# dalek-cryptography/zkp

Measured on AMD Instinct MI355X. Metric: proofs/sec + batch-verifies/sec, CMZ13 10-attr credential, 1/2/4/8 MI355X, higher is better.
Workload: dtype u32x9 (29-bit limbs, u64 accumulate)

## Files before the change

### zkp_amd/csrc/comb_tables.h

```cpp
#pragma once
#include "quad.h"
#include "stmt_pairs.h"

namespace zkp {

template <int TEETH>
struct comb_cfg {
  static_assert(TEETH == 4 || TEETH == 8 || TEETH == 16 || TEETH == 32, "teeth");
  static constexpr int BITS = 256 / TEETH;
  static constexpr int WINDOWS = BITS / 4;
  static constexpr int ENTRIES = 8 * TEETH + 1;
};
constexpr int comb_entries(int teeth) { return 8 * teeth + 1; }
constexpr int LADDER_ENTRIES = 8;

__device__ __forceinline__ void q_store_cached(dev_ext* dst, const qcached& c, int q) {
  uint32_t* w = reinterpret_cast<uint32_t*>(dst) + 9 * q;
#pragma unroll
  for (int i = 0; i < 9; ++i) w[i] = c.c.v[i];
}

__global__ void __launch_bounds__(256)
k_comb_slots(uint32_t n_points, const uint32_t* __restrict__ uses, uint32_t comb_min, uint32_t group_min, uint32_t max_tables,
             uint32_t* __restrict__ counter, uint32_t* __restrict__ slot_of, uint32_t* __restrict__ slot_pt, uint32_t* __restrict__ group_start,
             dev_affine* __restrict__ pts) {
  const uint32_t pi = blockIdx.x * blockDim.x + threadIdx.x;
  const uint32_t u = pi < n_points ? uses[pi] : 0u;
  const bool want = pi < n_points && u >= comb_min;
  const uint64_t mask = __ballot(want);
  if (!mask) return;
  const uint32_t lane = threadIdx.x & 63u;
  const int leader = __ffsll((long long)mask) - 1;
  const uint32_t gu = (want && u >= group_min) ? u : 0u;
  uint32_t incl = gu;
#pragma unroll
  for (int d = 1; d < 64; d <<= 1) {
    const uint32_t up = (uint32_t)__shfl_up((int)incl, d);
    if ((int)lane >= d) incl += up;
  }
  const uint32_t total = (uint32_t)__shfl((int)incl, 63);
  uint32_t base = 0, gbase = 0;
  if ((int)lane == leader) {
    base = atomicAdd(counter, (uint32_t)__popcll(mask));
    if (total) gbase = atomicAdd(counter + 1, total);
  }
  base = (uint32_t)__shfl((int)base, leader);
  gbase = (uint32_t)__shfl((int)gbase, leader);
  if (want) {
    const uint32_t slot = base + (uint32_t)__popcll(mask & ((1ull << lane) - 1ull));
    slot_of[pi] = slot < max_tables ? slot : 0xffffffffu;
    if (slot < max_tables) slot_pt[slot] = pi;
    else pts[pi].valid = 0;
    if (gu) group_start[pi] = gbase + incl - gu;
  }
}

template <int TEETH>
__global__ void __launch_bounds__(256, 2)
k_comb_tables(const uint32_t* __restrict__ n_slots, uint32_t max_tables, const uint32_t* __restrict__ slot_pt,
              const dev_affine* __restrict__ pts, dev_ext* __restrict__ comb) {
  using cfg = comb_cfg<TEETH>;
  const uint32_t gt = blockIdx.x * blockDim.x + threadIdx.x;
  const uint32_t slot = gt >> 2;
  const int q = (int)(gt & 3u);
  const uint32_t ns = min(*n_slots, max_tables);
  if (slot >= ns) return;
  const uint32_t pi = slot_pt[slot];
  if (pi & STMT_ABSORBED) return;
  qpt base;
  {
    const uint32_t* w = reinterpret_cast<const uint32_t*>(pts + pi);
    fe one;
    fe_1(one);
#pragma unroll
    for (int i = 0; i < 9; ++i) base.c.v[i] = q == 0 ? w[i] : (q == 1 ? w[9 + i] : (q == 3 ? w[18 + i] : one.v[i]));
  }
  dev_ext* tbl = comb + (size_t)slot * cfg::ENTRIES;
#pragma unroll 1
  for (int j = 0; j < TEETH; ++j) {
    qpt m2, m3, m4, m;
    qcached c1, c;
    q_to_cached(c1, base, q);
    q_store_cached(tbl + 8 * j + 0, c1, q);
    q_double(m2, base, q);
    q_to_cached(c, m2, q); q_store_cached(tbl + 8 * j + 1, c, q);
    q_add_cached(m3, m2, c1, q);
    q_to_cached(c, m3, q); q_store_cached(tbl + 8 * j + 2, c, q);
    q_double(m4, m2, q);
    q_to_cached(c, m4, q); q_store_cached(tbl + 8 * j + 3, c, q);
    q_add_cached(m, m4, c1, q);
    q_to_cached(c, m, q); q_store_cached(tbl + 8 * j + 4, c, q);
    q_double(m, m3, q);
    q_to_cached(c, m, q); q_store_cached(tbl + 8 * j + 5, c, q);
    q_add_cached(m, m, c1, q);
    q_to_cached(c, m, q); q_store_cached(tbl + 8 * j + 6, c, q);
    q_double(base, m4, q);
    q_to_cached(c, base, q); q_store_cached(tbl + 8 * j + 7, c, q);
#pragma unroll 1
    for (int d = 0; d < cfg::BITS - 3; ++d) q_double(base, base, q);
  }
  qcached c;
  q_to_cached(c, base, q);
  q_store_cached(tbl + 8 * TEETH, c, q);
}

__device__ __forceinline__ void store_comb_entry(dev_ext* dst, const ge_cached& c) {
  uint32_t w[36];
  fe_get(w, c.YmX); fe_get(w + 9, c.YpX); fe_get(w + 18, c.Z2); fe_get(w + 27, c.T2d);
  store_vec<9>(dst, w);
}
__device__ __forceinline__ void store_entries_staged(uint32_t (*stage)[64], const uint32_t* live, uint32_t lane, dev_ext* __restrict__ tbl0 ,
                                                     uint32_t entries_per_table, uint32_t e, const ge_cached& c) {
  uint32_t w[36];
  fe_get(w, c.YmX); fe_get(w + 9, c.YpX); fe_get(w + 18, c.Z2); fe_get(w + 27, c.T2d);
#pragma unroll
  for (int i = 0; i < 36; ++i) stage[i][lane] = w[i];
  __builtin_amdgcn_wave_barrier();
#pragma unroll
  for (int i = 0; i < 9; ++i) {
    const uint32_t ch = (uint32_t)i * 64u + lane, t = ch / 9u, q = ch - 9u * t;
    if (live[t]) {
      const uint4 v = make_uint4(stage[4 * q][t], stage[4 * q + 1][t], stage[4 * q + 2][t], stage[4 * q + 3][t]);
      reinterpret_cast<uint4*>(tbl0 + (size_t)t * entries_per_table + e)[q] = v;
    }
  }
  __builtin_amdgcn_wave_barrier();
}
template <int TEETH>
__device__ __forceinline__ void comb_table_lane(uint32_t slot, const uint32_t* __restrict__ n_slots, uint32_t max_tables, const uint32_t* __restrict__ slot_pt,
                                                const dev_affine* __restrict__ pts, dev_ext* __restrict__ comb) {
  using cfg = comb_cfg<TEETH>;
  const uint32_t ns = min(*n_slots, max_tables);
  if (slot >= ns) return;
  if (slot_pt[slot] & STMT_ABSORBED) return;
  ge_p3 base;
  load_affine(base, pts + slot_pt[slot]);
  dev_ext* tbl = comb + (size_t)slot * cfg::ENTRIES;
#pragma unroll 1
  for (int j = 0; j < TEETH; ++j) {
    ge_p3 m2, m3, m4, m;
    ge_cached c1, c;
    ge_to_cached(c1, base);
    store_comb_entry(tbl + 8 * j + 0, c1);
    ge_double<true>(m2, base);
    ge_to_cached(c, m2); store_comb_entry(tbl + 8 * j + 1, c);
    ge_add_cached(m3, m2, c1);
    ge_to_cached(c, m3); store_comb_entry(tbl + 8 * j + 2, c);
    ge_double<true>(m4, m2);
    ge_to_cached(c, m4); store_comb_entry(tbl + 8 * j + 3, c);
    ge_add_cached(m, m4, c1);
    ge_to_cached(c, m); store_comb_entry(tbl + 8 * j + 4, c);
    ge_double<true>(m, m3);
    ge_to_cached(c, m); store_comb_entry(tbl + 8 * j + 5, c);
    ge_add_cached(m, m, c1);
    ge_to_cached(c, m); store_comb_entry(tbl + 8 * j + 6, c);
    ge_double<true>(base, m4);
    ge_to_cached(c, base); store_comb_entry(tbl + 8 * j + 7, c);
#pragma unroll 1
    for (int d = 0; d < cfg::BITS - 4; ++d) ge_double<false>(base, base);
    ge_double<true>(base, base);
  }
  ge_cached c;
  ge_to_cached(c, base);
  store_comb_entry(tbl + 8 * TEETH, c);
}
template <int TEETH>
__global__ void __launch_bounds__(256, 2)
k_comb_tables_lane(const uint32_t* __restrict__ n_slots, uint32_t max_tables, const uint32_t* __restrict__ slot_pt,
                   const dev_affine* __restrict__ pts, dev_ext* __restrict__ comb) {
  comb_table_lane<TEETH>(blockIdx.x * blockDim.x + threadIdx.x, n_slots, max_tables, slot_pt, pts, comb);
}


template <int TEETH>
__device__ __forceinline__ void comb_table_pc(uint32_t slot0, const uint32_t* __restrict__ n_slots, uint32_t max_tables, const uint32_t* __restrict__ slot_pt,
                                              const dev_affine* __restrict__ pts, dev_ext* __restrict__ comb, uint32_t* hand) {
  using cfg = comb_cfg<TEETH>;
  const uint32_t wave = threadIdx.x >> 6, lane = threadIdx.x & 63u;
  const uint32_t ns = min(*n_slots, max_tables);
  const uint32_t slot = slot0 + lane;
  const bool have = slot < ns && !(slot_pt[slot < ns ? slot : 0u] & STMT_ABSORBED);
  dev_ext* tbl = comb + (size_t)(have ? slot : 0u) * cfg::ENTRIES;
  if (wave == 0) {
    ge_p3 base;
    ge_identity(base);
    if (have) load_affine(base, pts + slot_pt[slot]);
#pragma unroll 1
    for (int j = 0; j < TEETH; ++j) {
      uint32_t* h = hand + (j & 1) * 36 * 64 + lane;
#pragma unroll
      for (int i = 0; i < 9; ++i) { h[64 * i] = base.X.v[i]; h[64 * (9 + i)] = base.Y.v[i]; h[64 * (18 + i)] = base.Z.v[i]; h[64 * (27 + i)] = base.T.v[i]; }
      __syncthreads();
#pragma unroll 1
      for (int d = 0; d < cfg::BITS - 1; ++d) ge_double<false>(base, base);
      ge_double<true>(base, base);
    }
    if (have) {
      ge_cached c;
      ge_to_cached(c, base);
      store_comb_entry(tbl + 8 * TEETH, c);
    }
  } else {
#pragma unroll 1
    for (int j = 0; j < TEETH; ++j) {
      __syncthreads();
      const uint32_t* h = hand + (j & 1) * 36 * 64 + lane;
      ge_p3 base, m2, m3, m4, m;
#pragma unroll
      for (int i = 0; i < 9; ++i) { base.X.v[i] = h[64 * i]; base.Y.v[i] = h[64 * (9 + i)]; base.Z.v[i] = h[64 * (18 + i)]; base.T.v[i] = h[64 * (27 + i)]; }
      FE_TRACK(fe_set_ub_tight(base.X); fe_set_ub_tight(base.Y); fe_set_ub_tight(base.Z); fe_set_ub_tight(base.T));
      ge_cached c1, c;
      ge_to_cached(c1, base);
      ge_double<true>(m2, base);
      ge_add_cached(m3, m2, c1);
      ge_double<true>(m4, m2);
      if (have) {
        store_comb_entry(tbl + 8 * j + 0, c1);
        ge_to_cached(c, m2); store_comb_entry(tbl + 8 * j + 1, c);
        ge_to_cached(c, m3); store_comb_entry(tbl + 8 * j + 2, c);
        ge_to_cached(c, m4); store_comb_entry(tbl + 8 * j + 3, c);
      }
      ge_add_cached(m, m4, c1);
      if (have) { ge_to_cached(c, m); store_comb_entry(tbl + 8 * j + 4, c); }
      ge_double<true>(m, m3);
      if (have) { ge_to_cached(c, m); store_comb_entry(tbl + 8 * j + 5, c); }
      ge_add_cached(m, m, c1);
      if (have) { ge_to_cached(c, m); store_comb_entry(tbl + 8 * j + 6, c); }
      ge_double<true>(m, m4);
      if (have) { ge_to_cached(c, m); store_comb_entry(tbl + 8 * j + 7, c); }
    }
  }
}

__device__ __forceinline__ void load_comb_entry(ge_cached& c, const dev_ext* src) {
  uint32_t w[36];
  load_vec<9>(w, src);
  fe_set(c.YmX, w); fe_set(c.YpX, w + 9); fe_set(c.Z2, w + 18); fe_set(c.T2d, w + 27);
}

template <bool CT>
__device__ __forceinline__ void comb_select(ge_cached& sel, const dev_ext* __restrict__ row, uint32_t mag) {
  ge_cached_identity(sel);
  if (CT) {
#pragma unroll 1
    for (uint32_t h = 0; h < 4; ++h) {
      ge_cached c0, c1;
      load_comb_entry(c0, row + 2 * h + 0);
      load_comb_entry(c1, row + 2 * h + 1);
      ge_cached_cmov(sel, c0, (uint32_t)(mag == 2 * h + 1));
      ge_cached_cmov(sel, c1, (uint32_t)(mag == 2 * h + 2));
    }
  } else if (mag) {
    load_comb_entry(sel, row + (mag - 1));
  }
}

template <bool CT, int TEETH>
__device__ __forceinline__ void term_comb(uint32_t t, const uint8_t* __restrict__ scalars, const dev_ext* __restrict__ tbl,
                                          dev_ext* __restrict__ partial, uint32_t* ecol, bool no_carry = false) {
  using cfg = comb_cfg<TEETH>;
  uint32_t s[8], e[8], top;
  load_vec<2>(s, scalars + 32 * (size_t)t);
  sc_add_pattern(e, top, s, 0x88888888u);
#pragma unroll
  for (int j = 0; j < 8; ++j) ecol[256 * j] = e[j];
  ge_p3 acc;
  ge_identity(acc);
  if (CT) {
    ge_cached n0, n1;
    load_comb_entry(n0, tbl + 0);
    load_comb_entry(n1, tbl + 1);
#pragma unroll 1
    for (int w = cfg::WINDOWS - 1; w >= 0; --w) {
      if (w != cfg::WINDOWS - 1) {
        ge_double4_flat(acc);
      }
#pragma unroll 1
      for (int j = 0; j < TEETH; ++j) {
        const int nidx = j * cfg::WINDOWS + w;
        const uint32_t nib = (ecol[256 * (nidx >> 3)] >> (4 * (nidx & 7))) & 15u;
        const uint32_t neg = (uint32_t)(nib < 8u);
        const uint32_t mag = neg ? 8u - nib : nib - 8u;
        const dev_ext* row = tbl + 8 * j;
        ge_cached sel;
        ge_cached_identity(sel);
        ge_cached_cmov(sel, n0, (uint32_t)(mag == 1));
        ge_cached_cmov(sel, n1, (uint32_t)(mag == 2));
#pragma unroll 1
        for (uint32_t h = 1; h < 4; ++h) {
          ge_cached c0, c1;
          load_comb_entry(c0, row + 2 * h + 0);
          load_comb_entry(c1, row + 2 * h + 1);
          ge_cached_cmov(sel, c0, (uint32_t)(mag == 2 * h + 1));
          ge_cached_cmov(sel, c1, (uint32_t)(mag == 2 * h + 2));
        }
        const dev_ext* next = (j + 1 < TEETH) ? row + 8 : tbl;
        load_comb_entry(n0, next + 0);
        load_comb_entry(n1, next + 1);
        ge_cached_cneg(sel, neg);
        if (w == cfg::WINDOWS - 1 && j == 0) ge_from_cached(acc, sel);
        else ge_add_cached(acc, acc, sel);
      }
    }
  } else {
#pragma unroll 1
    for (int w = cfg::WINDOWS - 1; w >= 0; --w) {
      if (w != cfg::WINDOWS - 1) {
        ge_double4(acc);
      }
#pragma unroll 1
      for (int j = 0; j < TEETH; ++j) {
        const int nidx = j * cfg::WINDOWS + w;
        const uint32_t nib = (ecol[256 * (nidx >> 3)] >> (4 * (nidx & 7))) & 15u;
        const uint32_t neg = (uint32_t)(nib < 8u);
        const uint32_t mag = neg ? 8u - nib : nib - 8u;
        ge_cached sel;
        comb_select<false>(sel, tbl + 8 * j, mag);
        ge_cached_cneg(sel, neg);
        if (w == cfg::WINDOWS - 1 && j == 0) ge_from_cached(acc, sel);
        else ge_add_cached(acc, acc, sel);
      }
    }
  }
  if (!no_carry) {
    ge_cached sel, c;
    ge_cached_identity(sel);
    load_comb_entry(c, tbl + 8 * TEETH);
    ge_cached_cmov(sel, c, top);
    ge_add_cached(acc, acc, sel);
  }
  store_ext(partial + t, acc);
}

__device__ __forceinline__ void ge_p3_dpp_from(ge_p3& r, const ge_p3& a, int ctrl_sel) {
  if (ctrl_sel == 0) { fe_dpp<ZKP_QP(1, 1, 3, 3)>(r.X, a.X); fe_dpp<ZKP_QP(1, 1, 3, 3)>(r.Y, a.Y); fe_dpp<ZKP_QP(1, 1, 3, 3)>(r.Z, a.Z); fe_dpp<ZKP_QP(1, 1, 3, 3)>(r.T, a.T); }
  else { fe_dpp<ZKP_QP(2, 2, 2, 2)>(r.X, a.X); fe_dpp<ZKP_QP(2, 2, 2, 2)>(r.Y, a.Y); fe_dpp<ZKP_QP(2, 2, 2, 2)>(r.Z, a.Z); fe_dpp<ZKP_QP(2, 2, 2, 2)>(r.T, a.T); }
}
template <int TEETH>
__device__ __forceinline__ void term_comb_split4(uint32_t t, uint32_t q, const uint8_t* __restrict__ scalars, const dev_ext* __restrict__ comb, uint32_t slot,
                                                 dev_ext* __restrict__ partial, uint32_t* ecol, bool no_carry = false) {
  using cfg = comb_cfg<TEETH>;
  static_assert(cfg::WINDOWS == 4, "one lane of the quad per window");
  typedef __attribute__((address_space(3))) volatile uint32_t lds_word;
  lds_word* stash = (lds_word*)(ecol + 256 * 8);
  stash[0] = slot;
  stash[256] = t;
  const dev_ext* __restrict__ tbl = comb + (size_t)slot * cfg::ENTRIES;
  uint32_t s[8], e[8], top;
  load_vec<2>(s, scalars + 32 * (size_t)t);
  sc_add_pattern(e, top, s, 0x88888888u);
#pragma unroll
  for (int j = 0; j < 8; ++j) ecol[256 * j] = e[j];
  stash[512] = top;
  ge_p3 acc;
  ge_identity(acc);
  {
    ge_cached n0, n1;
    load_comb_entry(n0, tbl + 0);
    load_comb_entry(n1, tbl + 1);
#pragma unroll 1
    for (int j = 0; j < TEETH; ++j) {
      const uint32_t nidx = (uint32_t)j * cfg::WINDOWS + q;
      const uint32_t nib = (ecol[256 * (nidx >> 3)] >> (4 * (nidx & 7))) & 15u;
      const uint32_t neg = (uint32_t)(nib < 8u);
      const uint32_t mag = neg ? 8u - nib : nib - 8u;
      const dev_ext* row = tbl + 8 * j;
      ge_cached sel;
      ge_cached_identity(sel);
      ge_cached_cmov(sel, n0, (uint32_t)(mag == 1));
      ge_cached_cmov(sel, n1, (uint32_t)(mag == 2));
#pragma unroll 1
      for (uint32_t h = 1; h < 4; ++h) {
        ge_cached c0, c1;
        load_comb_entry(c0, row + 2 * h + 0);
        load_comb_entry(c1, row + 2 * h + 1);
        ge_cached_cmov(sel, c0, (uint32_t)(mag == 2 * h + 1));
        ge_cached_cmov(sel, c1, (uint32_t)(mag == 2 * h + 2));
      }
      const dev_ext* next = (j + 1 < TEETH) ? row + 8 : tbl;
      load_comb_entry(n0, next + 0);
      load_comb_entry(n1, next + 1);
      ge_cached_cneg(sel, neg);
      if (j == 0) ge_from_cached(acc, sel);
      else ge_add_cached(acc, acc, sel);
    }
  }
  {
    ge_p3 d = acc;
    ge_double4(d);
    fe_pick(acc.X, d.X, (q & 1u) != 0); fe_pick(acc.Y, d.Y, (q & 1u) != 0); fe_pick(acc.Z, d.Z, (q & 1u) != 0); fe_pick(acc.T, d.T, (q & 1u) != 0);
    ge_p3 o;
    ge_p3_dpp_from(o, acc, 0);
    ge_cached c;
    ge_to_cached(c, o);
    ge_add_cached(d, acc, c);
    fe_pick(acc.X, d.X, (q & 1u) == 0); fe_pick(acc.Y, d.Y, (q & 1u) == 0); fe_pick(acc.Z, d.Z, (q & 1u) == 0); fe_pick(acc.T, d.T, (q & 1u) == 0);
    d = acc;
    ge_double4(d);
    ge_double4(d);
    fe_pick(acc.X, d.X, q == 2u); fe_pick(acc.Y, d.Y, q == 2u); fe_pick(acc.Z, d.Z, q == 2u); fe_pick(acc.T, d.T, q == 2u);
    ge_p3_dpp_from(o, acc, 1);
    ge_to_cached(c, o);
    ge_add_cached(d, acc, c);
    fe_pick(acc.X, d.X, q == 0u); fe_pick(acc.Y, d.Y, q == 0u); fe_pick(acc.Z, d.Z, q == 0u); fe_pick(acc.T, d.T, q == 0u);
  }
  if (!no_carry) {
    ge_cached sel, c;
    ge_cached_identity(sel);
    load_comb_entry(c, comb + (size_t)stash[0] * cfg::ENTRIES + 8 * TEETH);
    ge_cached_cmov(sel, c, stash[512]);
    ge_add_cached(acc, acc, sel);
  }
  if (q == 0u) store_ext(partial + stash[256], acc);
}

constexpr int GROUP_RUNS = 3, GROUP_ROW_CHUNKS = 8 * 9, GROUP_IDENT_ROW = GROUP_RUNS * GROUP_ROW_CHUNKS, GROUP_CHUNK_ROWS = GROUP_IDENT_ROW + 9;
constexpr int GROUP_LDS_UINT4 = GROUP_CHUNK_ROWS * 16 + (256 + 16 * GROUP_RUNS) / 4;
static_assert(GROUP_MIN_USES >= 8, "a column of 16 consecutive grouped terms must span at most GROUP_RUNS points");

__device__ __forceinline__ void comb_group_block(uint32_t i0, uint32_t n_g, const uint32_t* __restrict__ list_g, const uint8_t* __restrict__ scalars,
                                                 const uint32_t* __restrict__ pidx, const uint32_t* __restrict__ slot_of,
                                                 const dev_ext* __restrict__ comb, dev_ext* __restrict__ partial, uint4* lds) {
  using cfg = comb_cfg<16>;
  constexpr uint32_t NONE = 0xffffffffu;
  const uint32_t tid = threadIdx.x, col = tid & 15u, k = tid >> 4;
  const uint32_t i = i0 + col * 16 + k;
  const bool listed = i < n_g;
  uint32_t t = 0, slot = NONE;
  if (listed) { t = list_g[i]; slot = slot_of[pidx[t]]; }
  uint32_t* slots = reinterpret_cast<uint32_t*>(lds + GROUP_CHUNK_ROWS * 16);
  uint32_t* colslot = slots + 256;
  slots[k * 16 + col] = slot;
  if (k < (uint32_t)GROUP_RUNS) colslot[col * GROUP_RUNS + k] = NONE;
  if (k < 9) {
    uint32_t w[36];
#pragma unroll
    for (int q = 0; q < 36; ++q) w[q] = (q == 0 || q == 9) ? 1u : (q == 18 ? 2u : 0u);
    uint4 v = make_uint4(0, 0, 0, 0);
#pragma unroll
    for (int q = 0; q < 9; ++q) if (k == (uint32_t)q) v = make_uint4(w[4 * q], w[4 * q + 1], w[4 * q + 2], w[4 * q + 3]);
    lds[(GROUP_IDENT_ROW + k) * 16 + col] = v;
  }
  __syncthreads();
  uint32_t run = 0;
  bool first = true;
#pragma unroll
  for (uint32_t kk = 1; kk < 16; ++kk) {
    const bool change = slots[kk * 16 + col] != slots[(kk - 1) * 16 + col];
    if (kk <= k) { run += change ? 1u : 0u; if (kk == k) first = change; }
  }
  if (first && run < (uint32_t)GROUP_RUNS) colslot[col * GROUP_RUNS + run] = slot;
  __syncthreads();
  const bool live = listed && slot != NONE && run < (uint32_t)GROUP_RUNS;
  const uint4* src[GROUP_RUNS];
  bool have[GROUP_RUNS];
#pragma unroll
  for (int r = 0; r < GROUP_RUNS; ++r) {
    const uint32_t sr = colslot[col * GROUP_RUNS + r];
    have[r] = sr != NONE;
    src[r] = reinterpret_cast<const uint4*>(comb + (size_t)(have[r] ? sr : 0u) * cfg::ENTRIES) + k;
  }
  const bool tail = k < (uint32_t)(GROUP_ROW_CHUNKS - 64);
  typedef __attribute__((address_space(1))) const void* gptr_t;
  typedef __attribute__((address_space(3))) void* lptr_t;
  const uint32_t wave = (uint32_t)__builtin_amdgcn_readfirstlane((int)(tid >> 6));
  auto issue = [&](uint32_t row) {
#pragma unroll
    for (int r = 0; r < GROUP_RUNS; ++r) {
      const uint4* p = src[r] + (size_t)row * GROUP_ROW_CHUNKS;
      uint4* d = lds + (size_t)(r * GROUP_ROW_CHUNKS + 4 * wave) * 16;
#pragma unroll
      for (int m = 0; m < 4; ++m)
        if (have[r]) __builtin_amdgcn_global_load_lds((gptr_t)(p + 16 * m), (lptr_t)(d + 16 * 16 * m), 16, 0, 0);
      if (have[r] && tail) __builtin_amdgcn_global_load_lds((gptr_t)(p + 64), (lptr_t)(d + 16 * 64), 16, 0, 0);
    }
  };
  uint32_t dlo[cfg::WINDOWS], dhi[cfg::WINDOWS], top = 0;
  {
    uint32_t sc[8], e[8];
#pragma unroll
    for (int q = 0; q < 8; ++q) sc[q] = 0;
    if (live) load_vec<2>(sc, scalars + 32 * (size_t)t);
    sc_add_pattern(e, top, sc, 0x88888888u);
#pragma unroll
    for (int w = 0; w < cfg::WINDOWS; ++w) {
      uint32_t lo = 0, hi = 0;
#pragma unroll
      for (int m = 0; m < 4; ++m) {
        lo |= (((e[m] >> (4 * w)) & 0xfu) | ((e[m] >> (12 + 4 * w)) & 0xf0u)) << (8 * m);
        hi |= (((e[m + 4] >> (4 * w)) & 0xfu) | ((e[m + 4] >> (12 + 4 * w)) & 0xf0u)) << (8 * m);
      }
      dlo[w] = lo; dhi[w] = hi;
    }
  }
  ge_p3 acc, lo;
  ge_identity(acc);
  ge_identity(lo);
  issue(0);
  auto pick = [&](uint32_t& c0, uint32_t& c1, ge_cached& sel, uint32_t& neg) {
    const uint32_t nib = c0 & 15u;
    c0 = __builtin_amdgcn_alignbit(c1, c0, 4);
    c1 >>= 4;
    neg = (uint32_t)(nib < 8u);
    const uint32_t mag = neg ? 8u - nib : nib - 8u;
    const uint32_t row = mag ? run * GROUP_ROW_CHUNKS + (mag - 1u) * 9u : (uint32_t)GROUP_IDENT_ROW;
    const uint4* ent = lds + (size_t)row * 16 + col;
    uint32_t wd[36];
#pragma unroll
    for (int q = 0; q < 9; ++q) {
      const uint4 x = ent[q * 16];
      wd[4 * q + 0] = x.x; wd[4 * q + 1] = x.y; wd[4 * q + 2] = x.z; wd[4 * q + 3] = x.w;
    }
    fe_set(sel.YmX, wd); fe_set(sel.YpX, wd + 9); fe_set(sel.Z2, wd + 18); fe_set(sel.T2d, wd + 27);
  };
#pragma unroll 1
  for (int pass = 0; pass < 2; ++pass) {
    if (live && pass) { ge_double4(acc); ge_double4(lo); }
    uint32_t alo = pass ? dlo[2] : dlo[3], ahi = pass ? dhi[2] : dhi[3];
    uint32_t blo = pass ? dlo[0] : dlo[1], bhi = pass ? dhi[0] : dhi[1];
#pragma unroll 1
    for (int j = 0; j < 16; ++j) {
      asm volatile("s_waitcnt vmcnt(0)\n\ts_barrier" ::: "memory");
      ge_cached sel;
      uint32_t neg = 0;
      const bool first = pass == 0 && j == 0;
      if (live) {
        pick(alo, ahi, sel, neg);
        ge_cached_cneg(sel, neg);
        if (first) ge_from_cached(acc, sel);
        else ge_add_cached(acc, acc, sel);
        pick(blo, bhi, sel, neg);
      }
      lds_barrier();
      if (pass == 0 || j != 15) issue((uint32_t)((j + 1) & 15));
      if (live) {
        ge_cached_cneg(sel, neg);
        if (first) ge_from_cached(lo, sel);
        else ge_add_cached(lo, lo, sel);
      }
    }
  }
  if (live) {
    ge_double4(acc);
    ge_double4(acc);
    ge_cached c;
    ge_to_cached(c, lo);
    ge_add_cached(acc, acc, c);
  }
  if (live) {
    ge_cached sel, c;
    ge_cached_identity(sel);
    load_comb_entry(c, comb + (size_t)slot * cfg::ENTRIES + 8 * 16);
    ge_cached_cmov(sel, c, top);
    ge_add_cached(acc, acc, sel);
    store_ext(partial + t, acc);
  }
}

constexpr uint32_t XBAR_RUNS = 8;
constexpr uint32_t XBAR_HALF_TERMS = 31, XBAR_WAVE_TERMS = 2 * XBAR_HALF_TERMS, XBAR_BLOCK_TERMS = 4 * XBAR_WAVE_TERMS;
constexpr int XBAR_WAVE_UINT4 = 9 * 64;
constexpr int XBAR_LDS_UINT4 = 4 * XBAR_WAVE_UINT4;
static_assert(2 + (XBAR_WAVE_TERMS - 2) / GROUP_MIN_USES <= XBAR_RUNS, "a wavefront's consecutive grouped terms must span at most XBAR_RUNS points");
static_assert(2 + (XBAR_HALF_TERMS - 2) / GROUP_MIN_USES <= 4 && XBAR_HALF_TERMS <= 32,
              "the terms of one crossbar service group (a half of the wavefront) must span at most 4 points: sources 32 lanes apart never meet");

__device__ __forceinline__ void comb_group_xbar(uint32_t i0, uint32_t n_g, const uint32_t* __restrict__ list_g, const uint8_t* __restrict__ scalars,
                                                const uint32_t* __restrict__ pidx, const uint32_t* __restrict__ slot_of,
                                                const dev_ext* __restrict__ comb, dev_ext* __restrict__ partial, uint4* lds, bool no_carry = false) {
  using cfg = comb_cfg<16>;
  constexpr uint32_t NONE = 0xffffffffu;
  const uint32_t tid = threadIdx.x, lane = tid & 63u;
  const uint32_t wave = (uint32_t)__builtin_amdgcn_readfirstlane((int)(tid >> 6));
  if (i0 + wave * XBAR_WAVE_TERMS >= n_g) return;
  const uint32_t hl = lane & 31u;
  const uint32_t i = i0 + wave * XBAR_WAVE_TERMS + (lane >> 5) * XBAR_HALF_TERMS + hl;
  const bool listed = hl < XBAR_HALF_TERMS && i < n_g;
  uint32_t t = 0, slot = NONE;
  if (listed) { t = list_g[i]; slot = slot_of[pidx[t]]; }
  uint32_t cur = slot;
  const uint32_t left = (uint32_t)__shfl_up((int)cur, 1);
  if (hl == 31u) cur = left;
  const uint32_t before = (uint32_t)__shfl_up((int)cur, 1);
  const bool change = lane == 0u || (listed && slot != before);
  const uint64_t cm = __ballot(change);
  const uint32_t run = (uint32_t)__popcll(cm & ((2ull << lane) - 1ull)) - 1u;
  const bool live = listed && slot != NONE && run < XBAR_RUNS;
  int first = -1;
  {
    uint64_t mm = cm;
#pragma unroll
    for (uint32_t r = 0; r < XBAR_RUNS; ++r) {
      const int f = mm ? (int)__ffsll((long long)mm) - 1 : -1;
      if ((lane >> 3) == r) first = f;
      mm &= mm - 1ull;
    }
  }
  uint32_t hslot = (uint32_t)__shfl((int)slot, first < 0 ? 0 : first);
  if (first < 0) hslot = NONE;
  const bool have = hslot != NONE;
  const uint4* hsrc = reinterpret_cast<const uint4*>(comb + (size_t)(have ? hslot : 0u) * cfg::ENTRIES + (lane & 7u));
  typedef __attribute__((address_space(1))) const void* gptr_t;
  typedef __attribute__((address_space(3))) void* lptr_t;
  uint4* wlds = lds + (size_t)wave * XBAR_WAVE_UINT4;
  const uint4* mine = wlds + lane;
  auto issue = [&](uint32_t row) {
    const uint4* p = hsrc + (size_t)row * (8 * 9);
    if (have) {
#pragma unroll
      for (int q = 0; q < 9; ++q) __builtin_amdgcn_global_load_lds((gptr_t)(p + q), (lptr_t)(wlds + 64 * q), 16, 0, 0);
    }
  };
  uint32_t dlo[cfg::WINDOWS], dhi[cfg::WINDOWS], top = 0;
  {
    uint32_t sc[8], e[8];
#pragma unroll
    for (int q = 0; q < 8; ++q) sc[q] = 0;
    if (live) load_vec<2>(sc, scalars + 32 * (size_t)t);
    sc_add_pattern(e, top, sc, 0x88888888u);
#pragma unroll
    for (int w = 0; w < cfg::WINDOWS; ++w) {
      uint32_t lo = 0, hi = 0;
#pragma unroll
      for (int m = 0; m < 4; ++m) {
        lo |= (((e[m] >> (4 * w)) & 0xfu) | ((e[m] >> (12 + 4 * w)) & 0xf0u)) << (8 * m);
        hi |= (((e[m + 4] >> (4 * w)) & 0xfu) | ((e[m + 4] >> (12 + 4 * w)) & 0xf0u)) << (8 * m);
      }
      dlo[w] = lo; dhi[w] = hi;
    }
  }
  ge_p3 acc, lo;
  ge_identity(acc);
  ge_identity(lo);
  issue(0);
  const uint32_t run8 = (run & (XBAR_RUNS - 1u)) * 8u;
  auto pick = [&](uint32_t& c0, uint32_t& c1, ge_cached& sel, uint32_t& neg) {
    const uint32_t nib = c0 & 15u;
    c0 = __builtin_amdgcn_alignbit(c1, c0, 4);
    c1 >>= 4;
    neg = (uint32_t)(nib < 8u);
    const uint32_t mag = neg ? 8u - nib : nib - 8u;
    const uint32_t nz = (uint32_t)(mag != 0u);
    const int src = (int)((run8 + mag - nz) << 2);
    uint32_t wd[36];
#pragma unroll
    for (int q = 0; q < 9; ++q) {
      const uint4 x = mine[q * 64];
      wd[4 * q + 0] = xbar_fetch(src, x.x); wd[4 * q + 1] = xbar_fetch(src, x.y);
      wd[4 * q + 2] = xbar_fetch(src, x.z); wd[4 * q + 3] = xbar_fetch(src, x.w);
    }
    const uint32_t m = 0u - nz, id = nz ^ 1u;
#pragma unroll
    for (int q = 0; q < 36; ++q) wd[q] &= m;
    wd[0] |= id; wd[9] |= id; wd[18] |= id << 1;
    fe_set(sel.YmX, wd); fe_set(sel.YpX, wd + 9); fe_set(sel.Z2, wd + 18); fe_set(sel.T2d, wd + 27);
  };
#pragma unroll 1
  for (int pass = 0; pass < 2; ++pass) {
    if (pass) { ge_double4(acc); ge_double4(lo); }
    uint32_t alo = pass ? dlo[2] : dlo[3], ahi = pass ? dhi[2] : dhi[3];
    uint32_t blo = pass ? dlo[0] : dlo[1], bhi = pass ? dhi[0] : dhi[1];
#pragma unroll 1
    for (int j = 0; j < 16; ++j) {
      asm volatile("s_waitcnt vmcnt(0)" ::: "memory");
      ge_cached sel;
      uint32_t neg = 0;
      const bool first = pass == 0 && j == 0;
      pick(alo, ahi, sel, neg);
      ge_cached_cneg(sel, neg);
      if (first) ge_from_cached(acc, sel);
      else ge_add_cached(acc, acc, sel);
      pick(blo, bhi, sel, neg);
      asm volatile("s_waitcnt lgkmcnt(0)" ::: "memory");
      if (pass == 0 || j != 15) issue((uint32_t)((j + 1) & 15));
      ge_cached_cneg(sel, neg);
      if (first) ge_from_cached(lo, sel);
      else ge_add_cached(lo, lo, sel);
    }
  }
  ge_double4(acc);
  ge_double4(acc);
  {
    ge_cached c;
    ge_to_cached(c, lo);
    ge_add_cached(acc, acc, c);
  }
  if (live && !no_carry) {
    ge_cached sel, c;
    ge_cached_identity(sel);
    load_comb_entry(c, comb + (size_t)slot * cfg::ENTRIES + 8 * 16);
    ge_cached_cmov(sel, c, top);
    ge_add_cached(acc, acc, sel);
  }
  if (live) store_ext(partial + t, acc);
}

constexpr uint32_t LADDER_GROUP_UINT4 = 64u * LADDER_ENTRIES * 9u;
__device__ __forceinline__ void ladder_store_entry(uint4* __restrict__ g, int e, const ge_cached& c) {
  uint32_t w[36];
  fe_get(w, c.YmX); fe_get(w + 9, c.YpX); fe_get(w + 18, c.Z2); fe_get(w + 27, c.T2d);
#pragma unroll
  for (int q = 0; q < 9; ++q) g[(9 * e + q) * 64] = make_uint4(w[4 * q], w[4 * q + 1], w[4 * q + 2], w[4 * q + 3]);
}
__device__ __forceinline__ void ladder_load_entry(ge_cached& c, const uint4* __restrict__ g, uint32_t e) {
  uint32_t w[36];
#pragma unroll
  for (int q = 0; q < 9; ++q) {
    const uint4 v = g[(9u * e + (uint32_t)q) * 64u];
    w[4 * q] = v.x; w[4 * q + 1] = v.y; w[4 * q + 2] = v.z; w[4 * q + 3] = v.w;
  }
  fe_set(c.YmX, w); fe_set(c.YpX, w + 9); fe_set(c.Z2, w + 18); fe_set(c.T2d, w + 27);
}
template <bool CT>
__device__ __forceinline__ void ladder_select(ge_cached& sel, const uint4* __restrict__ g, uint32_t mag) {
  ge_cached_identity(sel);
  if (CT) {
#pragma unroll 1
    for (uint32_t h = 0; h < 4; ++h) {
      ge_cached c0, c1;
      ladder_load_entry(c0, g, 2 * h + 0);
      ladder_load_entry(c1, g, 2 * h + 1);
      ge_cached_cmov(sel, c0, (uint32_t)(mag == 2 * h + 1));
      ge_cached_cmov(sel, c1, (uint32_t)(mag == 2 * h + 2));
    }
  } else if (mag) {
    ladder_load_entry(sel, g, mag - 1);
  }
}

template <bool CT>
__device__ __forceinline__ void term_ladder16(uint32_t t, const uint8_t* __restrict__ scalars, const dev_affine* __restrict__ pt,
                                              uint4* __restrict__ tbl , dev_ext* __restrict__ partial, uint32_t* ecol,
                                              bool no_carry = false) {
  uint32_t s[8], e[8], top;
  load_vec<2>(s, scalars + 32 * (size_t)t);
  sc_add_pattern(e, top, s, 0x88888888u);
#pragma unroll
  for (int j = 0; j < 8; ++j) ecol[256 * j] = e[j];
  ge_p3 acc;
  {
    ge_p3 P, m2, m3, m4, m;
    ge_cached c1, c;
    load_affine(P, pt);
    ge_to_cached(c1, P);
    ladder_store_entry(tbl, 0, c1);
    ge_double<true>(m2, P);
    ge_to_cached(c, m2); ladder_store_entry(tbl, 1, c);
    ge_add_cached(m3, m2, c1);
    ge_to_cached(c, m3); ladder_store_entry(tbl, 2, c);
    ge_double<true>(m4, m2);
    ge_to_cached(c, m4); ladder_store_entry(tbl, 3, c);
    ge_add_cached(m, m4, c1);
    ge_to_cached(c, m); ladder_store_entry(tbl, 4, c);
    ge_double<true>(m, m3);
    ge_to_cached(c, m); ladder_store_entry(tbl, 5, c);
    ge_add_cached(m, m, c1);
    ge_to_cached(c, m); ladder_store_entry(tbl, 6, c);
    ge_double<true>(m, m4);
    ge_to_cached(c, m); ladder_store_entry(tbl, 7, c);
    ge_identity(acc);
    if (!no_carry) {
      ge_cached sel;
      ge_cached_identity(sel);
      ge_cached_cmov(sel, c1, top);
      ge_from_cached(acc, sel);
    }
  }
#pragma unroll 1
  for (int j = 7; j >= 0; --j) {
    uint32_t cur = ecol[256 * j];
#pragma unroll 1
    for (int k = 0; k < 8; ++k) {
      ge_double4(acc);
      const uint32_t nib = cur >> 28;
      cur <<= 4;
      const uint32_t neg = (uint32_t)(nib < 8u);
      const uint32_t mag = neg ? 8u - nib : nib - 8u;
      ge_cached sel;
      ladder_select<CT>(sel, tbl, mag);
      ge_cached_cneg(sel, neg);
      ge_add_cached(acc, acc, sel);
    }
  }
  store_ext(partial + t, acc);
}

__global__ void __launch_bounds__(256, 2)
k_rider_tables(const uint32_t* __restrict__ n_slots, uint32_t max_tables, const uint32_t* __restrict__ slot_pt, const dev_affine* __restrict__ pts,
               dev_ext* __restrict__ comb) {
  __shared__ uint32_t stage[4][36][64];
  __shared__ uint32_t live[4][64];
  const uint32_t wave = threadIdx.x >> 6, lane = threadIdx.x & 63u;
  const uint32_t slot = blockIdx.x * blockDim.x + threadIdx.x, ns = min(*n_slots, max_tables);
  const uint32_t pi = slot < ns ? slot_pt[slot] : 0u;
  const bool have = slot < ns && (pi & STMT_ABSORBED);
  live[wave][lane] = have ? 1u : 0u;
  if (!__ballot(have)) return;
  ge_p3 P, m;
  ge_identity(P);
  if (have) load_affine(P, pts + (pi & ~STMT_ABSORBED));
  dev_ext* tbl0 = comb + (size_t)(slot - lane) * comb_cfg<16>::ENTRIES;
  ge_cached c1, c;
  ge_to_cached(c1, P);
  c = c1;
  m = P;
#pragma unroll 1
  for (int k = 0; k < 128; ++k) {
    if (k) {
      ge_add_cached(m, m, c1);
      ge_to_cached(c, m);
    }
    store_entries_staged(stage[wave], live[wave], lane, tbl0, comb_cfg<16>::ENTRIES, (uint32_t)k, c);
  }
}

__device__ __forceinline__ void ladder_build8(uint4* __restrict__ tbl, ge_cached& c1, const dev_affine* __restrict__ pt) {
  ge_p3 P, m2, m3, m4, m;
  ge_cached c;
  load_affine(P, pt);
  ge_to_cached(c1, P);
  ladder_store_entry(tbl, 0, c1);
  ge_double<true>(m2, P);
  ge_to_cached(c, m2); ladder_store_entry(tbl, 1, c);
  ge_add_cached(m3, m2, c1);
  ge_to_cached(c, m3); ladder_store_entry(tbl, 2, c);
  ge_double<true>(m4, m2);
  ge_to_cached(c, m4); ladder_store_entry(tbl, 3, c);
  ge_add_cached(m, m4, c1);
  ge_to_cached(c, m); ladder_store_entry(tbl, 4, c);
  ge_double<true>(m, m3);
  ge_to_cached(c, m); ladder_store_entry(tbl, 5, c);
  ge_add_cached(m, m, c1);
  ge_to_cached(c, m); ladder_store_entry(tbl, 6, c);
  ge_double<true>(m, m4);
  ge_to_cached(c, m); ladder_store_entry(tbl, 7, c);
}
__device__ __forceinline__ void term_ladder16_joint(uint32_t t, uint32_t t2, const uint8_t* __restrict__ scalars, const dev_affine* __restrict__ pt,
                                                    const dev_affine* __restrict__ pt2, uint4* __restrict__ tbl, uint4* __restrict__ tbl2,
                                                    const dev_ext* __restrict__ rider, dev_ext* __restrict__ partial, uint32_t* ecol) {
  uint32_t top, top2;
  {
    uint32_t s[8], e[8];
    load_vec<2>(s, scalars + 32 * (size_t)t);
    sc_add_pattern(e, top, s, 0x88888888u);
#pragma unroll
    for (int j = 0; j < 8; ++j) ecol[256 * j] = e[j];
    load_vec<2>(s, scalars + 32 * (size_t)t2);
    sc_add_pattern(e, top2, s, rider ? 0x80808080u : 0x88888888u);
#pragma unroll
    for (int j = 0; j < 8; ++j) ecol[256 * (8 + j)] = e[j];
  }
  ge_p3 acc;
  ge_identity(acc);
  {
    ge_cached c1;
    ladder_build8(tbl, c1, pt);
    if (top) ge_add_cached(acc, acc, c1);
    if (rider) load_comb_entry(c1, rider);
    else ladder_build8(tbl2, c1, pt2);
    if (top2) ge_add_cached(acc, acc, c1);
  }
#pragma unroll 1
  for (int j = 7; j >= 0; --j) {
    uint32_t cur = ecol[256 * j], cur2 = ecol[256 * (8 + j)];
#pragma unroll 1
    for (int k = 0; k < 8; ++k) {
      ge_double4(acc);
      uint32_t nib = cur >> 28;
      cur <<= 4;
      uint32_t neg = (uint32_t)(nib < 8u);
      uint32_t mag = neg ? 8u - nib : nib - 8u;
      ge_cached sel;
      ladder_select<false>(sel, tbl, mag);
      ge_cached_cneg(sel, neg);
      ge_add_cached(acc, acc, sel);
      if (rider) {
        if (k & 1) {
          const uint32_t v = cur2 >> 24;
          cur2 <<= 8;
          neg = (uint32_t)(v < 128u);
          mag = neg ? 128u - v : v - 128u;
          ge_cached_identity(sel);
          if (mag) load_comb_entry(sel, rider + (mag - 1u));
          ge_cached_cneg(sel, neg);
          ge_add_cached(acc, acc, sel);
        }
      } else {
        nib = cur2 >> 28;
        cur2 <<= 4;
        neg = (uint32_t)(nib < 8u);
        mag = neg ? 8u - nib : nib - 8u;
        ladder_select<false>(sel, tbl2, mag);
        ge_cached_cneg(sel, neg);
        ge_add_cached(acc, acc, sel);
      }
    }
  }
  store_ext(partial + t, acc);
  ge_identity(acc);
  store_ext(partial + t2, acc);
}

}
```

### zkp_amd/csrc/fused_flows.h

```cpp
#pragma once
#include "merlin_prog.h"
#include "transcript_kernels.h"

namespace zkp {

__global__ void __launch_bounds__(256)
k_wide_reduce(uint32_t n, const uint8_t* __restrict__ wide, uint8_t* __restrict__ out) {
  const uint32_t i = blockIdx.x * blockDim.x + threadIdx.x;
  if (i >= n) return;
  sc lo, hi, r;
  load_vec<2>(lo.v, wide + 64 * (size_t)i);
  load_vec<2>(hi.v, wide + 64 * (size_t)i + 32);
  sc_from_wide(r, lo, hi);
  store_vec<2>(out + 32 * (size_t)i, r.v);
}

__global__ void __launch_bounds__(256)
k_neg_reduce(uint32_t n, const uint8_t* in, uint8_t* out) {
  const uint32_t i = blockIdx.x * blockDim.x + threadIdx.x;
  if (i >= n) return;
  sc a, r;
  load_vec<2>(a.v, in + 32 * (size_t)i);
  sc_reduce(r, a);
  sc_neg(r, r);
// ... 835 lines not shown
  if (c->fused_plans.size() >= 64) free_fused_plans(c);
  *out = pl.get();
  c->fused_plans[key] = pl.release();
  return ZKP_OK;
}

#ifdef ZKP_BUILD_TEST_HOOKS
__global__ void k_noop(uint32_t* p) { if (p) *p = 0; }
#endif
bool transcript_single_lane(const zkp_ctx* c, uint32_t N, bool throughput) {
  return c->tr_lanes < 0 ? (throughput && N >= zkp_ctx::kVeryWideCallProofs) : c->tr_lanes == 1;
}
bool transcript_steps(const zkp_ctx* c, const prog_dev& p, uint32_t N, bool throughput, const uint64_t* d_img) {
  return c->tr_steps && p.steps && d_img && !transcript_single_lane(c, N, throughput);
}
void launch_assemble(zkp_ctx* c, const tr_steps_dev& sd, uint32_t N, const tr_bufs& bufs, uint64_t* d_img, uint32_t* d_failed) {
  const uint32_t rows = sd.n_img * 3u + ((sd.n_chk || (sd.tail >> 31)) ? 1u : 0u);
  if (rows) hipLaunchKernelGGL(k_transcript_assemble, dim3((N + TA_BLOCK - 1) / TA_BLOCK, rows), dim3(TA_BLOCK), 0, c->stream, sd, N, bufs, d_img, d_failed);
}
void run_program(zkp_ctx* c, const prog_dev& p_in, uint32_t N, const tr_bufs& bufs, uint8_t* d_ts, uint64_t* d_saved, uint32_t* d_failed, bool throughput,
                 uint64_t* d_img, bool owns_failed = false, int phase = 3) {
  if (!p_in.n) return;
  if (p_in.rg) {
    ZKP_SCHED(c, TR_LANES, 2);
    ZKP_SCHED(c, TR_STEPS, 0);
    prof_note(c, ZKP_K_TRANSCRIPT, "zkp::k_transcript_run_ragged");
    hipLaunchKernelGGL(k_transcript_run_ragged, dim3(p_in.rg_blocks), dim3(TR_BLOCK), 0, c->stream, p_in.rg, p_in.rg_idx, N, bufs, d_ts,
                       reinterpret_cast<uint32_t*>(d_saved), d_failed, owns_failed ? 0x80000000u : 0u);
    return;
  }
  prog_dev p = p_in;
  if (owns_failed) p.tail |= 0x80000000u;
  ZKP_SCHED(c, TR_LANES, transcript_single_lane(c, N, throughput) ? 1 : 2);
  ZKP_SCHED(c, TR_STEPS, transcript_steps(c, p, N, throughput, d_img));
  if (transcript_steps(c, p, N, throughput, d_img)) {
    prof_note(c, ZKP_K_TRANSCRIPT, "zkp::k_transcript_chain");
    tr_steps_dev sd = p.sd;
    sd.tail = p.tail;
    if (phase & 1) launch_assemble(c, sd, N, bufs, d_img, d_failed);
    constexpr uint32_t per_block = TR_BLOCK / 2;
    if (phase & 2) {
      if (throughput)
        hipLaunchKernelGGL(k_transcript_chain<false>, dim3((N + per_block - 1) / per_block), dim3(TR_BLOCK), 0, c->stream, sd, reinterpret_cast<const uint32_t*>(d_img), N, bufs, d_ts,
                           reinterpret_cast<uint32_t*>(d_saved));
      else
        hipLaunchKernelGGL(k_transcript_chain<true>, dim3((N + per_block - 1) / per_block), dim3(TR_BLOCK), 0, c->stream, sd, reinterpret_cast<const uint32_t*>(d_img), N, bufs, d_ts,
                           reinterpret_cast<uint32_t*>(d_saved));
    }
    return;
  }
  prof_note(c, ZKP_K_TRANSCRIPT, transcript_single_lane(c, N, throughput) ? "zkp::k_transcript_run1" : "zkp::k_transcript_run");
  if (transcript_single_lane(c, N, throughput)) {
    hipLaunchKernelGGL(k_transcript_run1, dim3((N + TR_BLOCK - 1) / TR_BLOCK), dim3(TR_BLOCK), 0, c->stream, p.ops, p.n, p.tables, N, bufs, d_ts, d_saved, d_failed, p.tail);
  } else {
    constexpr uint32_t per_block = TR_BLOCK / 2;
    hipLaunchKernelGGL(k_transcript_run, dim3((N + per_block - 1) / per_block), dim3(TR_BLOCK), 0, c->stream, p.ops, p.n, p.tables, N, bufs, d_ts,
                       reinterpret_cast<uint32_t*>(d_saved), d_failed, p.tail);
  }
}
void offer_program(zkp_ctx* c, const prog_dev& p, uint32_t N, const tr_bufs& bufs, uint8_t* d_ts, uint64_t* d_saved, uint32_t* d_failed, bool throughput, bool overlap,
                   uint64_t* d_img) {
  auto& t = c->pending_tr;
  const bool fuse = c->fuse_tables_transcript < 0 ? N < zkp_ctx::kVeryWideCallProofs : c->fuse_tables_transcript != 0;
  t.offered = t.active = fuse && p.n != 0 && !p.rg && throughput && !overlap && !transcript_single_lane(c, N, throughput);
  t.ops = p.ops; t.n_ops = p.n; t.tables = p.tables; t.N = N; t.bufs = bufs; t.ts = d_ts; t.saved = reinterpret_cast<uint32_t*>(d_saved); t.failed = d_failed; t.tail = p.tail;
  t.steps = transcript_steps(c, p, N, throughput, d_img);
  t.sd = p.sd; t.sd.tail = p.tail; t.img = d_img;
  if (p.n) {
    ZKP_SCHED(c, TR_LANES, transcript_single_lane(c, N, throughput) ? 1 : 2);
    ZKP_SCHED(c, TR_STEPS, t.steps);
  }
}
void run_program_pending(zkp_ctx* c, const prog_dev& p, uint32_t N, const tr_bufs& bufs, uint8_t* d_ts, uint64_t* d_saved, uint32_t* d_failed, bool throughput,
                         uint64_t* d_img) {
  const bool taken = c->pending_tr.offered && !c->pending_tr.active;
  if (p.n) ZKP_SCHED(c, FUSE_TT, taken);
  c->pending_tr.offered = c->pending_tr.active = false;
  if (!taken) run_program(c, p, N, bufs, d_ts, d_saved, d_failed, throughput, d_img);
}

inline bool side_forks(const zkp_ctx* c, bool overlap) {
  static const bool one_queue = [] { const char* e = getenv("GPU_MAX_HW_QUEUES"); return e && atoi(e) == 1; }();
  return overlap && !(c->capturing && one_queue);
}
int side_begin(zkp_ctx* c, hipStream_t* main_out, bool overlap) {
  *main_out = c->stream;
  overlap = side_forks(c, overlap);
  if (!overlap) return ZKP_OK;
  if (!c->side_stream) {
    HIP_TRY(hipStreamCreateWithFlags(&c->side_stream, hipStreamNonBlocking));
    HIP_TRY(hipEventCreateWithFlags(&c->ev_fork, hipEventDisableTiming));
    HIP_TRY(hipEventCreateWithFlags(&c->ev_join, hipEventDisableTiming));
  }
  HIP_TRY(hipEventRecord(c->ev_fork, c->stream));
  HIP_TRY(hipStreamWaitEvent(c->side_stream, c->ev_fork, 0));
  c->stream = c->side_stream;
  c->prof_suspended = true;
  return ZKP_OK;
}
int side_end(zkp_ctx* c, hipStream_t main, bool overlap) {
  if (!side_forks(c, overlap)) return ZKP_OK;
  c->prof_suspended = false;
  c->stream = main;
  HIP_TRY(hipEventRecord(c->ev_join, c->side_stream));
  return ZKP_OK;
}
int side_join(zkp_ctx* c, bool overlap) {
  if (side_forks(c, overlap)) HIP_TRY(hipStreamWaitEvent(c->stream, c->ev_join, 0));
  return ZKP_OK;
}

struct ws_view {
  char* base;
  uint8_t* u8(size_t o) const { return reinterpret_cast<uint8_t*>(base + o); }
  uint32_t* u32(size_t o) const { return reinterpret_cast<uint32_t*>(base + o); }
};

struct prove_inter { size_t saved, failed, wide, blind, off, sc, pidx, wchal, img, end; };
prove_inter prove_carve(const fused_plan& pl, size_t start) {
  const size_t N = pl.N, m = pl.s.m, nc = pl.s.nc, T = pl.T1;
  carve cv;
  cv.off = start;
  prove_inter o;
  o.saved = cv.take(N * 25 * 8);
  o.failed = cv.take(N * 4 + 4);
  o.wide = cv.take(N * m * 64 + 64);
  o.blind = cv.take(N * m * 32 + 32);
  o.off = cv.take((N * nc + 1) * 4);
  o.sc = cv.take(N * T * 32 + 32);
  o.pidx = cv.take(N * T * 4 + 4);
  o.wchal = cv.take(N * 64 + 64);
  o.img = cv.take(pl.img_bytes);
  o.end = cv.off;
  return o;
}
terms_cfg prove_terms_cfg(const zkp_ctx* c, const fused_plan& pl, bool throughput) {
  return cfg_from_terms(pl.tpt.data(), pl.T1, pl.s.ns, pl.s.np, pl.N, c->ct_comb_min(throughput, (size_t)pl.N * pl.T1));
}
int prove_core(zkp_ctx* c, const fused_plan& pl, const prove_inter& o, size_t ws_bound, uint8_t* d_ts, const uint8_t* d_sec, const uint8_t* d_tbl,
               const uint8_t* d_ent, uint8_t* d_chal, uint8_t* d_resp, uint8_t* d_coms, uint8_t* d_st8, bool overlap, bool throughput,
               const std::function<int()>* late_inputs = nullptr, const std::function<int()>* early_outputs = nullptr, bool late_early = false) {
  const uint32_t N = pl.N, m = pl.s.m, nc = pl.s.nc, T = pl.T1, n_points = pl.s.ns + pl.s.ni * N;
  const ws_view w{static_cast<char*>(c->ws)};
  tr_bufs hb{};
  hb.src[SRC_TABLE] = d_tbl; hb.src[SRC_SECRETS] = d_sec; hb.src[SRC_ENTROPY] = d_ent; hb.src[SRC_COMS] = d_coms;
  hb.dst[DST_WIDE] = w.u8(o.wide); hb.dst[DST_CHAL] = w.u8(o.wchal);
  uint64_t* d_saved = reinterpret_cast<uint64_t*>(w.base + o.saved);
  prof_begin(c);
  const size_t lanes = std::max<size_t>((size_t)N * T, (size_t)N * nc) + 1;
  terms_cfg tk = prove_terms_cfg(c, pl, throughput);
  if (o.end + terms_path_ws(n_points, N * T, N * nc, tk) > ws_bound)
    return fail(ZKP_ERR_ARG, "internal: prove_core's term path does not fit the workspace its caller sized");
  tk.throughput = throughput;
  if (pl.d_order) { tk.map.N = N; tk.map.nc = nc; tk.map.order = pl.d_order; }
  tk.stmt.toff = pl.d_tarr; tk.stmt.tpt = pl.d_tarr + nc + 1 + T; tk.stmt.N = N; tk.stmt.T = T; tk.stmt.nc = nc; tk.stmt.ns = pl.s.ns; tk.stmt.np = pl.s.np;
  tk.stmt.off = w.u32(o.off); tk.stmt.pidx = w.u32(o.pidx); tk.stmt.on = c->stmt_classify;
#ifdef ZKP_BUILD_TEST_HOOKS
  for (int q = 0; q < c->debug_dummy_launches; ++q) hipLaunchKernelGGL(k_noop, dim3(1), dim3(64), 0, c->stream, (uint32_t*)nullptr);
#endif
  uint64_t* d_img = pl.img_bytes ? reinterpret_cast<uint64_t*>(w.base + o.img) : nullptr;
  offer_program(c, pl.a, N, hb, d_ts, d_saved, w.u32(o.failed), throughput, overlap, d_img);
  {
    hipStream_t main;
    int rc = side_begin(c, &main, overlap);
    if (rc) { c->pending_tr.offered = c->pending_tr.active = false; return rc; }
    if (late_inputs && late_early) {
      hipStream_t cur = c->stream;
      c->stream = main;
      rc = (*late_inputs)();
      c->stream = cur;
      late_inputs = nullptr;
      if (rc) { (void)side_end(c, main, overlap); c->pending_tr.offered = c->pending_tr.active = false; return rc; }
    }
    if (!(nc && stmt_classify_applies(tk, N * T)))
      hipLaunchKernelGGL(k_stmt_index, grid1(lanes, 256), dim3(256), 0, c->stream, N, T, nc, pl.s.ns, pl.d_tarr, pl.d_tarr + nc + 1 + T, w.u32(o.off), w.u32(o.pidx));
    if (nc) rc = msm_terms_path(c, N * nc, w.u32(o.off), nullptr, w.u32(o.pidx), d_tbl, n_points, N * T, ZKP_CT, d_coms, d_st8, nullptr, o.end, false, PH_POINTS, tk);
    const int rc2 = side_end(c, main, overlap);
    if (rc || rc2) { c->pending_tr.offered = c->pending_tr.active = false; return rc ? rc : rc2; }
  }
  if (late_inputs) { const int rc = (*late_inputs)(); if (rc) return rc; }
  run_program_pending(c, pl.a, N, hb, d_ts, d_saved, w.u32(o.failed), throughput, d_img);
  prof_mark(c, ZKP_K_TRANSCRIPT);

  tk.prehalved = nc && terms_batched_encode(c, N * T, N * nc, tk.throughput);
  tk.canonical = true;
  if (m && std::max(m, T) <= 256) {
    const uint32_t P = 256 / std::max(m, T);
    hipLaunchKernelGGL(k_blind_scalars, dim3((N + P - 1) / P), dim3(256), 0, c->stream, N, T, m, P, pl.d_tarr + nc + 1, w.u8(o.wide), w.u8(o.blind), w.u8(o.sc),
                       tk.prehalved ? 1u : 0u);
  } else if (m) {
    hipLaunchKernelGGL(k_wide_reduce, grid1((size_t)N * m, 256), dim3(256), 0, c->stream, N * m, w.u8(o.wide), w.u8(o.blind));
    if (T) hipLaunchKernelGGL(k_stmt_scalars, grid1((size_t)N * T, 256), dim3(256), 0, c->stream, N, T, m, pl.d_tarr + nc + 1, w.u8(o.blind), (const uint8_t*)nullptr, w.u8(o.sc),
                              tk.prehalved ? 1u : 0u);
  }
  prof_mark(c, ZKP_K_SCALARS);
  HIP_TRY(hipGetLastError());
  {
    int rc = side_join(c, overlap);
    if (rc) return rc;
    if (nc) rc = msm_terms_path(c, N * nc, w.u32(o.off), w.u8(o.sc), w.u32(o.pidx), d_tbl, n_points, N * T, ZKP_CT, d_coms, d_st8, nullptr, o.end, false, PH_SCALARS, tk);
    if (rc) return rc;
    if (early_outputs) { rc = (*early_outputs)(); if (rc) return rc; }
  }
  run_program(c, pl.b, N, hb, d_ts, d_saved, w.u32(o.failed), throughput, d_img);
  prof_mark(c, ZKP_K_TRANSCRIPT);
  if (m && m <= 256) {
    const uint32_t P = 256 / m;
    hipLaunchKernelGGL(k_responses, dim3((N + P - 1) / P), dim3(256), 0, c->stream, N, m, P, d_sec, w.u8(o.wchal), d_chal, w.u8(o.blind), d_resp);
  } else {
    hipLaunchKernelGGL(k_wide_reduce, grid1(N, 256), dim3(256), 0, c->stream, N, w.u8(o.wchal), d_chal);
    if (m) hipLaunchKernelGGL(k_responses_wide, grid1((size_t)N * m, 256), dim3(256), 0, c->stream, N, m, d_sec, d_chal, w.u8(o.blind), d_resp);
  }
  prof_mark(c, ZKP_K_SCALARS);
  HIP_TRY(hipGetLastError());
  return ZKP_OK;
}

struct verify_inter { size_t failed, mc, off, sc, pidx, coms, st8, wchal, chal, img, end; };
verify_inter verify_carve(const fused_plan& pl, size_t start) {
  const size_t N = pl.N, nc = pl.s.nc, T1 = pl.T1;
  carve cv;
  cv.off = start;
  verify_inter o;
  o.failed = cv.take(N * 4 + 4);
  o.mc = cv.take(N * 32 + 32);
  o.off = cv.take((N * nc + 1) * 4);
  o.sc = cv.take(N * T1 * 32 + 32);
  o.pidx = cv.take(N * T1 * 4 + 4);
  o.coms = cv.take(N * nc * 32 + 32);
  o.st8 = cv.take(N * nc + 4);
  o.wchal = cv.take(N * 64 + 64);
  o.chal = cv.take(N * 32 + 32);
  o.img = cv.take(pl.img_bytes);
  o.end = cv.off;
  return o;
}
constexpr uint32_t kRiderLatencyProofs = 16384;
inline bool verify_riders(uint32_t N, bool throughput) { return throughput || N >= kRiderLatencyProofs; }
terms_cfg verify_terms_cfg(const zkp_ctx* c, const fused_plan& pl, bool riders = true) {
  const uint32_t N = pl.N, nc = pl.s.nc, T1 = pl.T1;
  terms_cfg tk = cfg_from_terms(pl.tpt.data(), T1, pl.s.ns, pl.s.np, N, 2);
  tk.stmt.toff = pl.d_tarr; tk.stmt.tpt = pl.d_tarr + nc + 1 + T1; tk.stmt.N = N; tk.stmt.T = T1; tk.stmt.nc = nc; tk.stmt.ns = pl.s.ns; tk.stmt.np = pl.s.np;
  tk.stmt.on = c->stmt_classify;
  if (c->joint_ladder && pl.d_pair && stmt_classify_applies(tk, N * T1)) {
    riders = riders && c->rider_tables;
    const terms_cfg paired = cfg_from_terms(pl.tpt.data(), T1, pl.s.ns, pl.s.np, N, 2, pl.pair.data(), riders);
    tk.max_tables = paired.max_tables; tk.max_ladder = paired.max_ladder; tk.teeth = paired.teeth;
    tk.stmt.pair = pl.d_pair;
    tk.rider_tables = riders;
  }
  return tk;
}
int verify_core(zkp_ctx* c, const fused_plan& pl, const verify_inter& o, size_t ws_bound, uint8_t* d_ts, const uint8_t* d_tbl, const uint8_t* d_claim,
                const uint8_t* d_resp, uint8_t* d_results, bool overlap, bool throughput, const std::function<int()>* late_inputs = nullptr, bool late_early = false) {
  const uint32_t N = pl.N, m = pl.s.m, nc = pl.s.nc, T1 = pl.T1, n_points = pl.s.ns + pl.s.ni * N;
  terms_cfg tk = verify_terms_cfg(c, pl, verify_riders(N, throughput));
  if (o.end + terms_path_ws(n_points, N * T1, N * nc, tk) > ws_bound)
    return fail(ZKP_ERR_ARG, "internal: verify_core's term path does not fit the workspace its caller sized");
  const ws_view w{static_cast<char*>(c->ws)};
  tr_bufs hb{};
  hb.src[SRC_TABLE] = d_tbl; hb.src[SRC_COMS] = w.u8(o.coms);
  hb.dst[DST_CHAL] = w.u8(o.wchal);
  HIP_TRY(hipMemsetAsync(w.base + o.failed, 0, (size_t)N * 4, c->stream));
  prof_begin(c);
  const size_t lanes = std::max<size_t>((size_t)N * T1, (size_t)N * nc) + 1;
  tk.throughput = throughput;
  if (pl.d_order) { tk.map.N = N; tk.map.nc = nc; tk.map.order = pl.d_order; }
  tk.stmt.off = w.u32(o.off); tk.stmt.pidx = w.u32(o.pidx);
  uint64_t* d_img = pl.img_bytes ? reinterpret_cast<uint64_t*>(w.base + o.img) : nullptr;
  offer_program(c, pl.a, N, hb, d_ts, nullptr, w.u32(o.failed), throughput, overlap, d_img);
  {
    hipStream_t main;
    int rc = side_begin(c, &main, overlap);
    if (rc) { c->pending_tr.offered = c->pending_tr.active = false; return rc; }
    if (late_inputs && late_early) {
      hipStream_t cur = c->stream;
      c->stream = main;
      rc = (*late_inputs)();
      c->stream = cur;
      late_inputs = nullptr;
      if (rc) { (void)side_end(c, main, overlap); c->pending_tr.offered = c->pending_tr.active = false; return rc; }
    }
    if (!stmt_classify_applies(tk, N * T1))
      hipLaunchKernelGGL(k_stmt_index, grid1(lanes, 256), dim3(256), 0, c->stream, N, T1, nc, pl.s.ns, pl.d_tarr, pl.d_tarr + nc + 1 + T1, w.u32(o.off), w.u32(o.pidx));
    rc = msm_terms_path(c, N * nc, w.u32(o.off), nullptr, w.u32(o.pidx), d_tbl, n_points, N * T1, ZKP_VARTIME, w.u8(o.coms), w.u8(o.st8), nullptr, o.end, true, PH_POINTS, tk);
    const int rc2 = side_end(c, main, overlap);
    if (rc || rc2) { c->pending_tr.offered = c->pending_tr.active = false; return rc ? rc : rc2; }
  }
  if (late_inputs) { const int rc = (*late_inputs)(); if (rc) return rc; }
  run_program_pending(c, pl.a, N, hb, d_ts, nullptr, w.u32(o.failed), throughput, d_img);
  prof_mark(c, ZKP_K_TRANSCRIPT);
  hipLaunchKernelGGL(k_neg_reduce, grid1(N, 256), dim3(256), 0, c->stream, N, d_claim, w.u8(o.mc));
  if (T1) hipLaunchKernelGGL(k_stmt_scalars, grid1((size_t)N * T1, 256), dim3(256), 0, c->stream, N, T1, m, pl.d_tarr + nc + 1, d_resp, w.u8(o.mc), w.u8(o.sc), 0u);
  prof_mark(c, ZKP_K_SCALARS);
  HIP_TRY(hipGetLastError());
  int rc = side_join(c, overlap);
  if (rc) return rc;
  rc = msm_terms_path(c, N * nc, w.u32(o.off), w.u8(o.sc), w.u32(o.pidx), d_tbl, n_points, N * T1, ZKP_VARTIME, w.u8(o.coms), w.u8(o.st8), nullptr, o.end, true, PH_SCALARS, tk);
  if (rc) return rc;
  run_program(c, pl.b, N, hb, d_ts, nullptr, w.u32(o.failed), throughput, d_img);
  prof_mark(c, ZKP_K_TRANSCRIPT);
  hipLaunchKernelGGL(k_wide_reduce, grid1(N, 256), dim3(256), 0, c->stream, N, w.u8(o.wchal), w.u8(o.chal));
  hipLaunchKernelGGL(k_verify_finish, grid1(N, 256), dim3(256), 0, c->stream, N, nc, pl.s.ns, m, w.u8(o.chal), d_claim, d_resp, w.u8(o.st8), w.u32(o.failed),
                     reinterpret_cast<const dev_affine*>(w.base + o.end), pl.d_tarr + nc + 1 + 2 * (size_t)T1, (uint32_t)pl.s.unref.size(), d_results);
  prof_mark(c, ZKP_K_SCALARS);
  HIP_TRY(hipGetLastError());
  return ZKP_OK;
}

struct batch_inter { size_t sc, failed, flags, wchal, mc, part, img, end; };
batch_inter batch_carve(const fused_plan& pl, size_t start, uint32_t K = 1) {
  const size_t N = pl.N, ns = pl.s.ns, N_each = N / (K ? K : 1), total = (size_t)K * ns + ((size_t)pl.s.ni + pl.s.nc) * N, nblk = (size_t)K * ((N_each + 255) / 256);
  carve cv;
  cv.off = start;
  batch_inter o;
  o.sc = cv.take(total * 32 + 32);
  o.failed = cv.take(N * 4 + 4);
  o.flags = cv.take((size_t)K * 4);
  o.wchal = cv.take(N * 64 + 64);
  o.mc = cv.take(N * 32 + 32);
  o.part = cv.take((ns ? ns : 1) * (nblk ? nblk : 1) * 32);
  o.img = cv.take(pl.img_bytes);
  o.end = cv.off;
  return o;
}
size_t optional_many_ws(uint64_t n_each, uint32_t K) {
  switch (pick_c(n_each)) {
    case 7: return pip_ws<7>(n_each, K);
    case 10: return pip_ws<10>(n_each, K);
    case 11: return pip_ws<11>(n_each, K);
    default: return pip_ws<16>(n_each, K);
  }
}
int batch_core(zkp_ctx* c, const fused_plan& pl, const batch_inter& o, uint8_t* d_ts, uint8_t* d_pts, const uint8_t* d_coms,
               const uint8_t* d_resp, const uint8_t* d_w, uint8_t* d_out ,
               uint32_t* d_status , bool throughput, uint32_t K = 1,
               bool overlap = false, const std::function<int()>* late_ts = nullptr, const std::function<int()>* late_scalars = nullptr, bool late_early = false) {
  const uint32_t N = pl.N, nc = pl.s.nc, ns = pl.s.ns, ni = pl.s.ni, N_each = N / K;
// ... 434 lines not shown
```

### zkp_amd/csrc/sc25519.h

```cpp
#pragma once
#include <stdint.h>
#include "fe25519.h"

namespace zkp {

struct sc { uint32_t v[8]; };

ZKP_HD uint32_t sc_l(int i) {
  return i == 0 ? 0x5cf5d3edu : i == 1 ? 0x5812631au : i == 2 ? 0xa2f79cd6u : i == 3 ? 0x14def9deu : i == 4 ? 0x00000000u : i == 5 ? 0x00000000u : i == 6 ? 0x00000000u : 0x10000000u;
}
ZKP_HD uint32_t sc_rr(int i) {
  return i == 0 ? 0x449c0f01u : i == 1 ? 0xa40611e3u : i == 2 ? 0x68859347u : i == 3 ? 0xd00e1ba7u : i == 4 ? 0x17f5be65u : i == 5 ? 0xceec73d2u : i == 6 ? 0x7c309a3du : 0x0399411bu;
}
ZKP_HD uint32_t sc_r1(int i) {
  return i == 0 ? 0x8d98951du : i == 1 ? 0xd6ec3174u : i == 2 ? 0x737dcf70u : i == 3 ? 0xc6ef5bf4u : i == 4 ? 0xfffffffeu : i == 5 ? 0xffffffffu : i == 6 ? 0xffffffffu : 0x0fffffffu;
}
ZKP_HD uint32_t sc_half(int i) {
  return i == 0 ? 0x2e7ae9f6u : i == 1 ? 0x2c09318du : i == 2 ? 0x517bce6bu : i == 3 ? 0x0a6f7cefu : i == 7 ? 0x08000000u : 0u;
}
constexpr uint32_t SC_N0INV = 0x12547e1bu;

ZKP_HD void sc_zero(sc& r) {
#pragma unroll
  for (int i = 0; i < 8; ++i) r.v[i] = 0;
// ... 82 lines not shown
    w[i] = (uint32_t)c;
    c >>= 32;
    m >>= 32;
  }
  const uint32_t neg = 0u - (uint32_t)((w[7] >> 28) == 0);
  c = 0;
#pragma unroll
  for (int i = 0; i < 8; ++i) {
    c += (uint64_t)w[i] + (i < 4 ? sc_delta(i) & neg : 0u);
    r.v[i] = (uint32_t)c;
    c >>= 32;
  }
  r.v[7] -= ~neg & 0x10000000u;
}
ZKP_HD void sc_reduce_wide(sc& r, const uint32_t* x) {
  uint32_t L[8], H[9], y[13], L2[8], H2[5], z[9], v[9];
  sc_split252<9, true>(L, H, x);
  sc_mul_delta<9>(y, H);
  sc_split252<5, false>(L2, H2, y);
  sc_mul_delta<5>(z, H2);
  uint64_t c = 0, br = 0;
#pragma unroll
  for (int i = 0; i < 8; ++i) {
    const uint64_t t = (uint64_t)sc_l(i) - L2[i] - br;
    br = (t >> 63) & 1u;
    c += (uint64_t)L[i] + z[i] + (uint32_t)t;
    v[i] = (uint32_t)c;
    c >>= 32;
  }
  v[8] = (uint32_t)c + z[8];
  sc_reduce_tail(r, v);
}
ZKP_HD void sc_reduce_384(sc& r, const uint32_t* x) {
  uint32_t L[8], H[5], y[9], v[9];
  sc_split252<5, true>(L, H, x);
  sc_mul_delta<5>(y, H);
  uint64_t c = 0, br = 0;
#pragma unroll
  for (int i = 0; i < 9; ++i) {
    const uint64_t t = (uint64_t)sc_32l(i) - y[i] - br;
    br = (t >> 63) & 1u;
    c += (uint64_t)(i < 8 ? L[i] : 0u) + (uint32_t)t;
    v[i] = (uint32_t)c;
    c >>= 32;
  }
  sc_reduce_tail(r, v);
}

ZKP_HD void sc_muladd(sc& r, const sc& a, const sc& b, const sc& c) {
  uint32_t x[16];
  sc_mul_words<8, 8>(x, a.v, b.v, c.v);
  sc_reduce_wide(r, x);
}
ZKP_HD void sc_mul(sc& r, const sc& a, const sc& b) {
  uint32_t x[16];
  sc_mul_words<8, 8>(x, a.v, b.v);
  sc_reduce_wide(r, x);
}
ZKP_HD void sc_mul_u128(sc& r, const sc& a, const uint32_t w[4]) {
  uint32_t x[12];
  sc_mul_words<4, 8>(x, w, a.v);
  sc_reduce_384(r, x);
}
ZKP_HD void sc_reduce(sc& r, const sc& a) {
  uint32_t v[9];
#pragma unroll
  for (int i = 0; i < 8; ++i) v[i] = a.v[i];
  v[8] = 0;
  sc_reduce_tail(r, v);
}

ZKP_HD void sc_mont(sc& r, const sc& a, const sc& b) {
  uint32_t t[10];
#pragma unroll
  for (int i = 0; i < 10; ++i) t[i] = 0;
#pragma unroll
  for (int i = 0; i < 8; ++i) {
    uint64_t c = 0;
#pragma unroll
    for (int j = 0; j < 8; ++j) {
      c += (uint64_t)a.v[i] * b.v[j] + t[j];
      t[j] = (uint32_t)c;
      c >>= 32;
    }
    c += t[8];
    t[8] = (uint32_t)c;
    t[9] = (uint32_t)(c >> 32);
    const uint32_t m = t[0] * SC_N0INV;
    c = (uint64_t)m * sc_l(0) + t[0];
    c >>= 32;
#pragma unroll
    for (int j = 1; j < 4; ++j) {
      c += (uint64_t)m * sc_l(j) + t[j];
      t[j - 1] = (uint32_t)c;
      c >>= 32;
    }
#pragma unroll
    for (int j = 4; j < 7; ++j) {
      c += t[j];
      t[j - 1] = (uint32_t)c;
      c >>= 32;
    }
    c += ((uint64_t)m << 28) + t[7];
    t[6] = (uint32_t)c;
    c >>= 32;
    c += t[8];
    t[7] = (uint32_t)c;
    t[8] = t[9] + (uint32_t)(c >> 32);
  }
#pragma unroll
  for (int i = 0; i < 8; ++i) r.v[i] = t[i];
  sc_cond_sub_l(r);
}
ZKP_HD void sc_to_mont(sc& r, const sc& a) {
  sc rr;
#pragma unroll
  for (int i = 0; i < 8; ++i) rr.v[i] = sc_rr(i);
  sc_mont(r, a, rr);
}

ZKP_HD uint32_t sc_not_canonical(const uint32_t v[8]) {
  uint64_t br = 0;
#pragma unroll
  for (int i = 0; i < 8; ++i) br = (((uint64_t)v[i] - sc_l(i) - br) >> 63) & 1u;
  return br ? 0u : 1u;
}

ZKP_HD void sc_add_pattern(uint32_t e[8], uint32_t& top, const uint32_t s[8], uint32_t pattern) {
  uint64_t c = 0;
#pragma unroll
  for (int i = 0; i < 8; ++i) {
    c += (uint64_t)s[i] + pattern;
    e[i] = (uint32_t)c;
    c >>= 32;
  }
  top = (uint32_t)c;
}

ZKP_HD uint32_t sc_fold_sign(uint32_t s[8]) {
  uint32_t d[8];
  uint64_t b1 = 0, b2 = 0;
#pragma unroll
  for (int i = 0; i < 8; ++i) {
    const uint64_t t1 = (uint64_t)sc_half(i) - s[i] - b1;
    b1 = (t1 >> 63) & 1u;
    const uint64_t t2 = (uint64_t)sc_l(i) - s[i] - b2;
    d[i] = (uint32_t)t2;
    b2 = (t2 >> 63) & 1u;
  }
  const bool fold = b1 && !b2;
#pragma unroll
  for (int i = 0; i < 8; ++i) s[i] = fold ? d[i] : s[i];
  return fold ? 1u : 0u;
}

ZKP_HD void sc_halve(sc& r, const sc& a) {
  sc t;
  sc_reduce(t, a);
  const uint32_t odd = 0u - (t.v[0] & 1u);
  uint64_t c = 0;
  uint32_t w[8];
#pragma unroll
  for (int i = 0; i < 8; ++i) {
    c += (uint64_t)t.v[i] + (sc_l(i) & odd);
    w[i] = (uint32_t)c;
    c >>= 32;
  }
#pragma unroll
  for (int i = 0; i < 7; ++i) r.v[i] = (w[i] >> 1) | (w[i + 1] << 31);
  r.v[7] = w[7] >> 1;
}

ZKP_HD void sc_halve_canonical(sc& r, const sc& t) {
  const uint32_t odd = 0u - (t.v[0] & 1u);
  uint64_t c = 0;
  uint32_t w[8];
#pragma unroll
  for (int i = 0; i < 8; ++i) {
    c += (uint64_t)t.v[i] + (sc_l(i) & odd);
    w[i] = (uint32_t)c;
    c >>= 32;
  }
#pragma unroll
  for (int i = 0; i < 7; ++i) r.v[i] = (w[i] >> 1) | (w[i + 1] << 31);
  r.v[7] = w[7] >> 1;
}

ZKP_HD void sc_from_wide(sc& r, const sc& lo, const sc& hi) {
  uint32_t x[16];
#pragma unroll
  for (int i = 0; i < 8; ++i) { x[i] = lo.v[i]; x[8 + i] = hi.v[i]; }
  sc_reduce_wide(r, x);
}

ZKP_HD void sc_sqmul(sc& y, int n, const sc& t) {
#pragma unroll 1
  for (int k = 0; k < n; ++k) sc_mont(y, y, y);
  sc_mont(y, y, t);
}
ZKP_HD void sc_invert(sc& r, const sc& a) {
  sc y, a2, t3, t5, t7, t9, t11, t13, t15, one;
  sc_to_mont(y, a);
  sc_mont(a2, y, y);
  sc_mont(t3, a2, y);
  sc_mont(t5, a2, t3);
  sc_mont(t7, a2, t5);
  sc_mont(t9, a2, t7);
  sc_mont(t11, a2, t9);
  sc_mont(t13, a2, t11);
  sc_mont(t15, a2, t13);
  sc_sqmul(y, 130, t5);
  sc_sqmul(y, 6, t13);
  sc_sqmul(y, 3, t7);
  sc_sqmul(y, 5, t15);
  sc_sqmul(y, 4, t9);
  sc_sqmul(y, 4, t13);
  sc_sqmul(y, 3, t7);
  sc_sqmul(y, 4, t5);
  sc_sqmul(y, 7, t11);
  sc_sqmul(y, 4, t13);
  sc_sqmul(y, 3, t7);
  sc_sqmul(y, 5, t7);
  sc_sqmul(y, 6, t13);
  sc_sqmul(y, 3, t3);
  sc_sqmul(y, 6, t11);
  sc_sqmul(y, 10, t9);
  sc_sqmul(y, 4, t3);
  sc_sqmul(y, 5, t3);
  sc_sqmul(y, 7, t13);
  sc_sqmul(y, 6, t11);
  sc_sqmul(y, 4, t9);
  sc_sqmul(y, 3, t7);
  sc_sqmul(y, 5, t11);
  sc_sqmul(y, 3, t5);
  sc_sqmul(y, 6, t15);
  sc_sqmul(y, 3, t5);
  sc_sqmul(y, 3, t3);
  sc_zero(one);
  one.v[0] = 1;
  sc_mont(r, y, one);
}

}
```

### zkp_amd/csrc/transcript_kernels.h

```cpp
#pragma once
#include "merlin_prog.h"
#include "strobe_lane.h"
#include "comb_tables.h"

namespace zkp {

__device__ __forceinline__ uint32_t pair_swap(uint32_t v) {
  return (uint32_t)__builtin_amdgcn_update_dpp(0, (int)v, 0xB1 , 0xf, 0xf, true);
}
__device__ __forceinline__ uint32_t rotl_half(uint32_t mine, uint32_t partner, int R) {
  const int n = R & 31;
  if (R & 32) return n ? __builtin_amdgcn_alignbit(partner, mine, 32 - n) : partner;
  return n ? __builtin_amdgcn_alignbit(mine, partner, 32 - n) : mine;
}
__device__ __forceinline__ uint32_t half_of(uint64_t v, uint32_t h) { return h ? (uint32_t)(v >> 32) : (uint32_t)v; }

template <bool UNROLL = false>
__device__ __forceinline__ void keccak_f1600_split(uint32_t a[25], uint32_t h) {
  constexpr uint64_t RC[24] = {
      0x0000000000000001ULL, 0x0000000000008082ULL, 0x800000000000808aULL, 0x8000000080008000ULL, 0x000000000000808bULL,
      0x0000000080000001ULL, 0x8000000080008081ULL, 0x8000000000008009ULL, 0x000000000000008aULL, 0x0000000000000088ULL,
      0x0000000080008009ULL, 0x000000008000000aULL, 0x000000008000808bULL, 0x800000000000008bULL, 0x8000000000008089ULL,
      0x8000000000008003ULL, 0x8000000000008002ULL, 0x8000000000000080ULL, 0x000000000000800aULL, 0x800000008000000aULL,
      0x8000000080008081ULL, 0x8000000000008080ULL, 0x0000000080000001ULL, 0x8000000080008008ULL};
// ... 120 lines not shown
  const uint32_t j_raw = bid * (TR_BLOCK / 2) + ((threadIdx.x & (TR_BLOCK - 1)) >> 1);
  const bool live = j_raw < N;
  const uint32_t j = live ? j_raw : N - 1;
  transcript_pair_run(j, live, j_raw == 0, S, prog, n_ops, tables, N, bufs, ts, saved, failed, tail);
}

__global__ void __launch_bounds__(TR_BLOCK)
k_transcript_run(const tr_op* __restrict__ prog, uint32_t n_ops, const uint64_t* __restrict__ tables, uint32_t N, const tr_bufs bufs,
                 uint8_t* __restrict__ ts, uint32_t* __restrict__ saved , uint32_t* __restrict__ failed, uint32_t tail) {
  __shared__ uint32_t S[25 * TR_BLOCK];
  transcript_pair_block(blockIdx.x, S, prog, n_ops, tables, N, bufs, ts, saved, failed, tail);
}

struct tr_rg_block { const tr_op* ops; const uint64_t* tables; uint32_t n_ops, tail, first, count; };
static_assert(sizeof(tr_rg_block) == 32, "tr_rg_block layout");
__global__ void __launch_bounds__(TR_BLOCK)
k_transcript_run_ragged(const tr_rg_block* __restrict__ blocks, const uint32_t* __restrict__ idx, uint32_t N, const tr_bufs bufs, uint8_t* __restrict__ ts,
                        uint32_t* __restrict__ saved , uint32_t* __restrict__ failed, uint32_t owns_failed ) {
  __shared__ uint32_t S[25 * TR_BLOCK];
  const tr_rg_block b = blocks[blockIdx.x];
  const uint32_t p = (threadIdx.x & (TR_BLOCK - 1)) >> 1;
  const bool live = p < b.count;
  const uint32_t j = idx[b.first + (live ? p : b.count - 1)];
  transcript_pair_run(j, live, blockIdx.x == 0 && p == 0, S, b.ops, b.n_ops, b.tables, N, bufs, ts, saved, failed, b.tail | owns_failed);
}

struct tr_steps_dev {
  const tr_step* steps = nullptr;
  const tr_op* emit = nullptr;
  const tr_op* src = nullptr;
  const uint32_t* src_off = nullptr;
  const uint64_t* cx = nullptr;
  const uint32_t* keep32 = nullptr;
  const tr_op* chk = nullptr;
  uint32_t n_steps = 0, n_img = 0, n_chk = 0, tail = 0;
};

constexpr uint32_t TA_WORDS = 7, TA_BLOCK = 64;
__global__ void __launch_bounds__(TA_BLOCK)
k_transcript_assemble(const tr_steps_dev p, uint32_t N, const tr_bufs bufs, uint64_t* __restrict__ img, uint32_t* __restrict__ failed) {
  const uint32_t j = blockIdx.x * TA_BLOCK + threadIdx.x, y = blockIdx.y;
  if (j >= N) return;
  if (y < p.n_img * 3u) {
    const uint32_t k0 = (y / 3u) * 21u + (y % 3u) * TA_WORDS;
#pragma unroll 1
    for (uint32_t k = k0; k < k0 + TA_WORDS; ++k) {
      uint64_t x = p.cx[k];
      for (uint32_t q = p.src_off[k]; q < p.src_off[k + 1]; ++q) {
        const tr_op o = p.src[q];
        x ^= tr_src_word(tr_unpack(o.ctl, o.stride, o.off), bufs, j);
      }
      img[(size_t)k * N + j] = x;
    }
  } else {
    uint32_t bad = 0;
    for (uint32_t q = 0; q < p.n_chk; ++q) {
      const tr_op o = p.chk[q];
      const tr_fields f = tr_unpack(o.ctl, o.stride, o.off);
      const uint4* s = reinterpret_cast<const uint4*>(tr_src_ptr(bufs, f.src_buf - 1u) + (size_t)j * f.stride + f.off);
      const uint4 lo = s[0], hi = s[1];
      if ((lo.x | lo.y | lo.z | lo.w | hi.x | hi.y | hi.z | hi.w) == 0) bad = 1;
    }
    if (bad || (p.tail >> 31)) failed[j] = bad;
    if ((p.tail >> 31) && j == 0) failed[N] = 0;
  }
}

__device__ __forceinline__ void transcript_chain_block(uint32_t bid, uint32_t* S , const tr_steps_dev& p, const uint32_t* __restrict__ img32, uint32_t N,
                                                       const tr_bufs& bufs, uint8_t* __restrict__ ts, uint32_t* __restrict__ saved ) {
  const uint32_t lane = threadIdx.x & (TR_BLOCK - 1), h = lane & 1;
  const uint32_t j_raw = bid * (TR_BLOCK / 2) + (lane >> 1);
  const bool live = j_raw < N;
  const uint32_t j = live ? j_raw : N - 1;
  uint32_t* col = S + lane;
  uint32_t* blob = reinterpret_cast<uint32_t*>(ts + 208 * (size_t)j);
  uint32_t a[25], ni[21], nk[21];
#pragma unroll
  for (int i = 0; i < 25; ++i) a[i] = blob[2 * i + h];
  const size_t wstride = 2 * (size_t)N;
  const uint32_t* mycol = img32 + 2 * (size_t)j + h;
  uint32_t* sv = saved + 2 * (size_t)j + h;
  const uint32_t n_real = p.n_steps - 1;
  {
    const uint32_t im0 = p.steps[0].img;
#pragma unroll
    for (int k = 0; k < 21; ++k) { ni[k] = mycol[((size_t)im0 * 21 + k) * wstride]; nk[k] = p.keep32[(size_t)im0 * 42 + 2 * k + h]; }
  }
  constexpr uint32_t CH = TR_BLOCK - 1;
  for (uint32_t base = 0; base < n_real; base += CH) {
    const uint32_t cnt = n_real - base < CH ? n_real - base : CH;
    uint4 mine = make_uint4(0, 0, 0, 0);
    if (lane <= cnt) mine = reinterpret_cast<const uint4*>(p.steps)[base + lane];
    for (uint32_t i = 0; i < cnt; ++i) {
      const uint32_t fl = (uint32_t)__builtin_amdgcn_readlane((int)mine.x, (int)i);
      const uint32_t nim = (uint32_t)__builtin_amdgcn_readlane((int)mine.y, (int)(i + 1));
      if (fl & TS_RESTORE) {
#pragma unroll
        for (int k = 0; k < 25; ++k) a[k] = sv[k * wstride];
      }
      if (fl & TS_EMIT) {
        const uint32_t elo = (uint32_t)__builtin_amdgcn_readlane((int)mine.z, (int)i), en = (uint32_t)__builtin_amdgcn_readlane((int)mine.w, (int)i);
#pragma unroll
        for (int k = 0; k < 21; ++k) col[TR_BLOCK * k] = a[k];
        uint4 eo = make_uint4(0, 0, 0, 0);
        if (lane < en) eo = reinterpret_cast<const uint4*>(p.emit)[elo + lane];
        for (uint32_t q = 0; q < en; ++q) {
          const uint32_t o_ctl = (uint32_t)__builtin_amdgcn_readlane((int)eo.x, (int)q), o_stride = (uint32_t)__builtin_amdgcn_readlane((int)eo.y, (int)q);
          const uint64_t o_off = (uint32_t)__builtin_amdgcn_readlane((int)eo.z, (int)q) | (uint64_t)(uint32_t)__builtin_amdgcn_readlane((int)eo.w, (int)q) << 32;
          const tr_fields op = tr_unpack(o_ctl, o_stride, o_off);
          uint8_t* d = tr_dst_ptr(bufs, op.dst_buf - 1u) + (size_t)j * op.stride + op.off;
          const uint32_t lo = op.dlb > 4 * h ? op.dlb : 4 * h;
          const uint32_t hi = op.dlb + op.dnb < 4 * h + 4 ? op.dlb + op.dnb : 4 * h + 4;
          if (hi > lo && live) {
            const uint32_t v = col[TR_BLOCK * op.w] >> (8 * (lo - 4 * h));
            uint8_t* dp = d + (lo - op.dlb);
            if (hi - lo == 4) {
              __builtin_memcpy(dp, &v, 4);
            } else {
              for (uint32_t k = 0; k < hi - lo; ++k) dp[k] = (uint8_t)(v >> (8 * k));
            }
          }
        }
      }
#pragma unroll
      for (int k = 0; k < 21; ++k) a[k] = (uint32_t)__builtin_amdgcn_bitop3_b32((int)a[k], (int)nk[k], (int)ni[k], 0x6A);
#pragma unroll
      for (int k = 0; k < 21; ++k) { ni[k] = mycol[((size_t)nim * 21 + k) * wstride]; nk[k] = p.keep32[(size_t)nim * 42 + 2 * k + h]; }
      if (fl & TS_PERMUTE) keccak_f1600_split<true>(a, h);
      if ((fl & TS_SAVE) && live) {
#pragma unroll
        for (int k = 0; k < 25; ++k) sv[k * wstride] = a[k];
      }
    }
  }
  if (!live) return;
#pragma unroll
  for (int i = 0; i < 25; ++i) blob[2 * i + h] = a[i];
  if (h == 0) { blob[50] = p.tail & 0xffffffu; blob[51] = 0; }
}

template <bool ALONE>
__global__ void __launch_bounds__(TR_BLOCK)
k_transcript_chain(const tr_steps_dev p, const uint32_t* __restrict__ img32, uint32_t N, const tr_bufs bufs, uint8_t* __restrict__ ts, uint32_t* __restrict__ saved) {
  __shared__ uint32_t S[25 * TR_BLOCK];
  if constexpr (ALONE) asm volatile("" ::: "a239");
  transcript_chain_block(blockIdx.x, S, p, img32, N, bufs, ts, saved);
}

template <int TEETH>
__global__ void __launch_bounds__(2 * TR_BLOCK, 2)
k_tables_transcript_pc(uint32_t tr_blocks, const tr_op* __restrict__ prog, uint32_t n_ops, const uint64_t* __restrict__ tables, uint32_t N, const tr_bufs bufs,
                       uint8_t* __restrict__ ts, uint32_t* __restrict__ saved, uint32_t* __restrict__ failed, uint32_t tail,
                       const uint32_t* __restrict__ n_slots, uint32_t max_tables, const uint32_t* __restrict__ slot_pt,
                       const dev_affine* __restrict__ pts, dev_ext* __restrict__ comb) {
  __shared__ uint32_t S[2 * 36 * 64];
  static_assert(2 * 36 * 64 >= 2 * 25 * TR_BLOCK, "LDS of k_tables_transcript_pc");
  const uint32_t wave = threadIdx.x >> 6, trb = (tr_blocks + 1) / 2;
  if (blockIdx.x < trb) {
    const uint32_t bid = 2 * blockIdx.x + wave;
    if (bid < tr_blocks) transcript_pair_block(bid, S + wave * 25 * TR_BLOCK, prog, n_ops, tables, N, bufs, ts, saved, failed, tail);
  } else {
    comb_table_pc<TEETH>((blockIdx.x - trb) * 64u, n_slots, max_tables, slot_pt, pts, comb, S);
  }
}

template <int TEETH>
__global__ void __launch_bounds__(2 * TR_BLOCK, 2)
k_tables_chain_pc(uint32_t tr_blocks, const tr_steps_dev p, const uint32_t* __restrict__ img32, uint32_t N, const tr_bufs bufs, uint8_t* __restrict__ ts,
                  uint32_t* __restrict__ saved, const uint32_t* __restrict__ n_slots, uint32_t max_tables, const uint32_t* __restrict__ slot_pt,
                  const dev_affine* __restrict__ pts, dev_ext* __restrict__ comb) {
  __shared__ uint32_t S[2 * 36 * 64];
  const uint32_t wave = threadIdx.x >> 6, trb = (tr_blocks + 1) / 2;
  if (blockIdx.x < trb) {
    const uint32_t bid = 2 * blockIdx.x + wave;
    if (bid < tr_blocks) transcript_chain_block(bid, S + wave * 25 * TR_BLOCK, p, img32, N, bufs, ts, saved);
  } else {
    comb_table_pc<TEETH>((blockIdx.x - trb) * 64u, n_slots, max_tables, slot_pt, pts, comb, S);
  }
}

__global__ void __launch_bounds__(TR_BLOCK)
k_transcript_run1(const tr_op* __restrict__ prog, uint32_t n_ops, const uint64_t* __restrict__ tables, uint32_t N, const tr_bufs bufs,
                  uint8_t* __restrict__ ts, uint64_t* __restrict__ saved , uint32_t* __restrict__ failed, uint32_t tail) {
  __shared__ uint64_t S[25 * TR_BLOCK];
  const uint32_t lane = threadIdx.x;
  const uint32_t j_raw = blockIdx.x * TR_BLOCK + lane;
  const bool live = j_raw < N;
  const uint32_t j = live ? j_raw : N - 1;
  uint64_t* col = S + lane;
  uint64_t* blob = reinterpret_cast<uint64_t*>(ts + 208 * (size_t)j);
#pragma unroll
  for (int i = 0; i < 25; ++i) col[TR_BLOCK * i] = blob[i];
  uint32_t bad = 0;
  for (uint32_t base = 0; base < n_ops; base += TR_BLOCK) {
    const uint32_t cnt = n_ops - base < TR_BLOCK ? n_ops - base : TR_BLOCK;
    uint4 mine = make_uint4(0, 0, 0, 0);
    if (lane < cnt) mine = reinterpret_cast<const uint4*>(prog)[base + lane];
    for (uint32_t i = 0; i < cnt; ++i) {
      const uint32_t o_ctl = (uint32_t)__builtin_amdgcn_readlane((int)mine.x, (int)i);
      const uint32_t o_stride = (uint32_t)__builtin_amdgcn_readlane((int)mine.y, (int)i);
      const uint64_t o_off = (uint32_t)__builtin_amdgcn_readlane((int)mine.z, (int)i) | (uint64_t)(uint32_t)__builtin_amdgcn_readlane((int)mine.w, (int)i) << 32;
      tr_exec_op(tr_unpack(o_ctl, o_stride, o_off), tables, j, bufs, col, TR_BLOCK, saved + j, N, &bad, live);
    }
  }
  if (!live) return;
#pragma unroll
  for (int i = 0; i < 25; ++i) blob[i] = col[TR_BLOCK * i];
  blob[25] = tail & 0xffffffu;
  if (bad || (tail >> 31)) failed[j] = bad;
  if ((tail >> 31) && j_raw == 0) failed[N] = 0;
}

constexpr int STROBE_BLOCK = 64;

__device__ __forceinline__ void strobe_label_to_lds(uint64_t* lab, const strobe_label& label) {
  if (threadIdx.x == 0) {
#pragma unroll
    for (int i = 0; i < (int)STROBE_LABEL_WORDS; ++i) lab[i] = label.w[i];
  }
  __syncthreads();
}

__global__ void __launch_bounds__(STROBE_BLOCK)
k_strobe_append_csr(uint32_t N, uint32_t shared_initial, const uint8_t* ts_in, uint8_t* ts_out, const strobe_label label,
                    const uint8_t* __restrict__ msgs, uint64_t msgs_len, const uint64_t* __restrict__ offsets) {
  __shared__ uint64_t S[25 * STROBE_BLOCK];
  __shared__ uint64_t lab[STROBE_LABEL_WORDS];
  strobe_label_to_lds(lab, label);
  for (uint32_t j = blockIdx.x * STROBE_BLOCK + threadIdx.x; j < N; j += gridDim.x * STROBE_BLOCK) {
    strobe_lane L{S + threadIdx.x, STROBE_BLOCK, 0, 0, 0};
    uint64_t tail = strobe_load(L, reinterpret_cast<const uint64_t*>(ts_in + 208 * (size_t)(shared_initial ? 0u : j)));
    if (strobe_valid(L)) {
      uint64_t lo = offsets[j];
      const uint64_t len = sha512_clamp(lo, offsets[j + 1], msgs_len);
      strobe_append_message(L, lab, label.len, strobe_msg{msgs + lo, len}, len);
      tail = strobe_tail(L);
    }
    strobe_store(L, reinterpret_cast<uint64_t*>(ts_out + 208 * (size_t)j), tail);
  }
}

__global__ void __launch_bounds__(STROBE_BLOCK)
k_strobe_challenge(uint32_t N, uint8_t* __restrict__ ts, const strobe_label label, uint32_t len, uint8_t* __restrict__ out) {
  __shared__ uint64_t S[25 * STROBE_BLOCK];
  __shared__ uint64_t lab[STROBE_LABEL_WORDS];
  strobe_label_to_lds(lab, label);
  for (uint32_t j = blockIdx.x * STROBE_BLOCK + threadIdx.x; j < N; j += gridDim.x * STROBE_BLOCK) {
    strobe_lane L{S + threadIdx.x, STROBE_BLOCK, 0, 0, 0};
    uint64_t* blob = reinterpret_cast<uint64_t*>(ts + 208 * (size_t)j);
    uint8_t* o = out + (size_t)len * j;
    strobe_load(L, blob);
    if (strobe_valid(L)) {
      strobe_challenge_bytes(L, lab, label.len, strobe_out{o}, len);
      strobe_store(L, blob, strobe_tail(L));
    } else {
      for (uint32_t i = 0; i < len; ++i) o[i] = 0;
    }
  }
}

}
```

### zkp_amd/csrc/zkp_kernels.hip

```cpp
#include <hip/hip_runtime.h>
#include <sys/syscall.h>
#include <unistd.h>
#include <cctype>
#include <cstdio>
#include <cstring>
#include <algorithm>
#include <atomic>
#include <functional>
#include <map>
#include <memory>
#include <mutex>
#include <set>
#include <string>
#include <vector>
#include "../../include/zkp_mi355x.h"
#include "dev_layout.h"

using namespace zkp;

__device__ __forceinline__ uint32_t sel8(const uint32_t w[8], int j) {
  uint32_t r = w[0];
#pragma unroll
  for (int i = 1; i < 8; ++i) r = (j == i) ? w[i] : r;
  return r;
// ... 10 lines not shown
__global__ void __launch_bounds__(256, 2)
k_decode_affine(uint32_t n, const uint8_t* __restrict__ enc, dev_affine* __restrict__ out, const uint32_t* __restrict__ only) {
  const uint32_t i = blockIdx.x * blockDim.x + threadIdx.x;
  if (i >= n) return;
  if (only && !only[i]) { out[i].valid = 1; return; }
  uint32_t w[8];
  load_vec<2>(w, enc + 32 * (size_t)i);
  ge_p3 p;
  const uint32_t ok = ristretto_decode(p, w);
  store_affine(out + i, p, ok);
}

__device__ __forceinline__ void term_generic(uint32_t t, const uint8_t* __restrict__ scalars, const uint32_t* __restrict__ pidx,
                                             uint32_t n_points, const dev_affine* __restrict__ pts, dev_ext* __restrict__ partial) {
  uint32_t s[8], e[8], top;
  load_vec<2>(s, scalars + 32 * (size_t)t);
  sc_add_pattern(e, top, s, 0xAAAAAAAAu);
  ge_p3 P, P2, acc;
  const uint32_t pi = pidx[t];
  load_affine(P, pts + (pi < n_points ? pi : 0u));
  ge_cached c1, c2;
  ge_to_cached(c1, P);
  ge_double<true>(P2, P);
  ge_to_cached(c2, P2);
  ge_identity(acc);
  fe_cmov(acc.X, P.X, top);
  fe_cmov(acc.Y, P.Y, top);
  fe_cmov(acc.T, P.T, top);
#pragma unroll 1
  for (int j = 7; j >= 0; --j) {
    uint32_t cur = sel8(e, j);
#pragma unroll 1
    for (int k = 0; k < 16; ++k) {
      const uint32_t d = cur >> 30;
      cur <<= 2;
      ge_double<false>(acc, acc);
      ge_double<true>(acc, acc);
      const uint32_t neg = (uint32_t)(d < 2);
      const uint32_t mag = neg ? 2u - d : d - 2u;
      ge_cached sel;
      ge_cached_identity(sel);
      ge_cached_cmov(sel, c1, (uint32_t)(mag == 1));
      ge_cached_cmov(sel, c2, (uint32_t)(mag == 2));
      ge_cached_cneg(sel, neg);
      ge_add_cached(acc, acc, sel);
    }
  }
  store_ext(partial + t, acc);
}

__global__ void __launch_bounds__(256, 2)
k_terms_r4(uint32_t n_terms, const uint8_t* __restrict__ scalars, const uint32_t* __restrict__ pidx,
           uint32_t n_points, const dev_affine* __restrict__ pts, dev_ext* __restrict__ partial) {
  const uint32_t t = blockIdx.x * blockDim.x + threadIdx.x;
  if (t < n_terms) term_generic(t, scalars, pidx, n_points, pts, partial);
}

#ifdef ZKP_BUILD_TEST_HOOKS
__device__ uint64_t* g_wave_cycles = nullptr;
__device__ uint32_t g_wave_cycles_cap = 0;
#define ZKP_WAVE_T0 const uint64_t wave_t0_ = __builtin_readcyclecounter();
#define ZKP_WAVE_T1(cls) do { const uint64_t dt_ = __builtin_readcyclecounter() - wave_t0_; const uint32_t wi_ = blockIdx.x * 4 + (threadIdx.x >> 6); \
  if (g_wave_cycles && (threadIdx.x & 63u) == 0 && wi_ < g_wave_cycles_cap) g_wave_cycles[wi_] = ((uint64_t)(cls) << 56) | (dt_ & 0x00ffffffffffffffull); } while (0)
#else
#define ZKP_WAVE_T0
#define ZKP_WAVE_T1(cls)
#endif

enum : int { LOOKUP_XBAR = 0, LOOKUP_SCAN = 1, LOOKUP_LDS = 2 };
template <int LOOKUP>
constexpr int terms_lds_uint4() {
  if (LOOKUP == LOOKUP_XBAR) return XBAR_LDS_UINT4 > 512 ? XBAR_LDS_UINT4 : 512;
  return HOT_ROW_CHUNKS * HOT_COPIES > GROUP_LDS_UINT4 ? HOT_ROW_CHUNKS * HOT_COPIES : GROUP_LDS_UINT4;
}
template <bool CT, int TEETH, bool LADDER, int LOOKUP = LOOKUP_XBAR, bool SPLIT = false>
__global__ void __launch_bounds__(256, 2)
k_terms_split(const uint8_t* __restrict__ scalars, const uint32_t* __restrict__ pidx, uint32_t n_points,
              const dev_ext* __restrict__ comb, const uint32_t* __restrict__ slot_of, const uint32_t* __restrict__ class_start,
              const uint32_t* __restrict__ blk_start, const uint32_t* __restrict__ list, const dev_niels* __restrict__ tables,
              const dev_affine* __restrict__ pts, dev_ext* __restrict__ ladder_rw, uint32_t max_ladder, dev_ext* __restrict__ partial,
              uint32_t ladder_stride, const uint32_t* __restrict__ pair, uint32_t stmt_T, uint32_t no_carry) {
  static_assert(LOOKUP == LOOKUP_XBAR || HOT_LDS_ROWS, "7-bit fixed-base windows exist on the crossbar only");
  __shared__ uint4 hot_lds[terms_lds_uint4<LOOKUP>()];
  uint32_t* ecol = reinterpret_cast<uint32_t*>(hot_lds) + threadIdx.x;
  const uint32_t n_hot = class_start[CLASS_COMB], n_comb = class_start[CLASS_LADDER] - n_hot;
  const uint32_t n_ladder = LADDER ? class_start[CLASS_GROUP] - class_start[CLASS_LADDER] : 0u;
  const uint32_t n_group = (CT && TEETH == 16) ? class_start[HOT_CLASSES] - class_start[CLASS_GROUP] : 0u;
  const uint32_t ladder_blocks = (n_ladder + blockDim.x - 1) / blockDim.x;
  const uint32_t comb_lanes = SPLIT ? 4u * n_comb : n_comb;
  const uint32_t comb_blocks = (comb_lanes + blockDim.x - 1) / blockDim.x;
  const uint32_t group_terms = LOOKUP == LOOKUP_XBAR ? XBAR_BLOCK_TERMS : 256u;
  const uint32_t group_blocks = (n_group + group_terms - 1) / group_terms;
  uint32_t vb = blockIdx.x;
  if (LADDER && ladder_stride > 1) {
    const uint32_t q = blockIdx.x / ladder_stride, r = blockIdx.x - q * ladder_stride;
    if (r == 0 && q < ladder_blocks) vb = q;
    else vb = ladder_blocks + blockIdx.x - min((blockIdx.x + ladder_stride - 1) / ladder_stride, ladder_blocks);
  }
  ZKP_WAVE_T0
  if (LADDER && vb < ladder_blocks) {
    if constexpr (LADDER) {
      const uint32_t i = vb * blockDim.x + threadIdx.x;
      if (i < n_ladder && i < max_ladder) {
        const uint32_t t = list[n_hot + n_comb + i];
        const uint32_t pi = pidx[t];
        uint4* tbl = reinterpret_cast<uint4*>(ladder_rw) + (size_t)(i >> 6) * LADDER_GROUP_UINT4 + (i & 63u);
        bool joint = false;
        static_assert(CT || terms_lds_uint4<LOOKUP>() >= 1024, "variable-time ladder blocks need LDS for two recoded scalars");
        if constexpr (!CT && terms_lds_uint4<LOOKUP>() >= 1024) {
          const uint32_t k2 = pair ? pair[t % stmt_T] : STMT_UNPAIRED;
          if (k2 != STMT_UNPAIRED) {
            const uint32_t t2 = t - t % stmt_T + k2, i2 = i + ((max_ladder + 63u) & ~63u), pi2 = pidx[t2];
            const uint32_t s2 = slot_of[pi2];
            const dev_ext* rider = (s2 != 0xffffffffu && (s2 & STMT_ABSORBED)) ? comb + (size_t)(s2 & ~STMT_ABSORBED) * comb_cfg<16>::ENTRIES : nullptr;
            term_ladder16_joint(t, t2, scalars, pts + pi, pts + pi2, tbl, reinterpret_cast<uint4*>(ladder_rw) + (size_t)(i2 >> 6) * LADDER_GROUP_UINT4 + (i2 & 63u), rider, partial, ecol);
            joint = true;
          }
        }
        if (!joint) term_ladder16<CT>(t, scalars, pts + pi, tbl, partial, ecol, CT && no_carry);
      }
    }
    ZKP_WAVE_T1(1);
  } else if (vb < ladder_blocks + comb_blocks) {
    const uint32_t i = (vb - ladder_blocks) * blockDim.x + threadIdx.x;
    if constexpr (SPLIT) {
      {
        const uint32_t ti = i >> 2;
        if (ti < n_comb) {
          const uint32_t t = list[n_hot + ti];
          const uint32_t pi = pidx[t];
          if (pi < n_points) {
            const uint32_t slot = slot_of[pi];
            if (slot != 0xffffffffu) term_comb_split4<TEETH>(t, i & 3u, scalars, comb, slot, partial, ecol, CT && no_carry);
          }
        }
        ZKP_WAVE_T1(2);
        return;
      }
    }
    if (i < n_comb) {
      const uint32_t t = list[n_hot + i];
      const uint32_t pi = pidx[t];
      if (pi < n_points) {
        const uint32_t slot = slot_of[pi];
        if (slot != 0xffffffffu) term_comb<CT, TEETH>(t, scalars, comb + (size_t)slot * comb_cfg<TEETH>::ENTRIES, partial, ecol, CT && no_carry);
      }
    }
    ZKP_WAVE_T1(2);
  } else if (vb < ladder_blocks + comb_blocks + group_blocks) {
    if constexpr (CT && TEETH == 16) {
      if constexpr (LOOKUP == LOOKUP_XBAR)
        comb_group_xbar((vb - ladder_blocks - comb_blocks) * XBAR_BLOCK_TERMS, n_group, list + class_start[CLASS_GROUP], scalars, pidx, slot_of, comb, partial, hot_lds, no_carry != 0);
      else
        comb_group_block((vb - ladder_blocks - comb_blocks) * 256u, n_group, list + class_start[CLASS_GROUP], scalars, pidx, slot_of, comb, partial, hot_lds);
    }
    ZKP_WAVE_T1(3);
  } else {
    const uint32_t hb = vb - ladder_blocks - comb_blocks - group_blocks;
    if (hb >= blk_start[HOT_SLOTS]) return;
    uint32_t c = 0;
    while (blk_start[c + 1] <= hb) ++c;
    const uint4* src = reinterpret_cast<const uint4*>(tables + (size_t)c * HOT_SLOT_NIELS);
    const uint32_t i = (hb - blk_start[c]) * 256 + threadIdx.x;
    const bool live = i < class_start[c + 1] - class_start[c];
    const uint32_t t = live ? list[class_start[c] + i] : 0u;
    uint32_t s[8], e[9];
    ge_p3 acc;
    ge_identity(acc);
    if constexpr (LOOKUP == LOOKUP_XBAR) {
      if (hb * 256u + (threadIdx.x & ~63u) - blk_start[c] * 256u >= class_start[c + 1] - class_start[c]) return;
#pragma unroll
      for (int q = 0; q < 8; ++q) s[q] = 0;
      if (live) load_vec<2>(s, scalars + 32 * (size_t)t);
      const bool fold = CT && no_carry;
      uint32_t flip = 0;
      if (fold) flip = sc_fold_sign(s);
      hot_recode(e, s, fold);
      fixed_base_xbar(acc, e, src, fold);
      if (fold) ge_cneg(acc, flip);
    } else {
      if (live) {
        load_vec<2>(s, scalars + 32 * (size_t)t);
        hot_recode(e, s);
      }
      fixed_base_block<LOOKUP == LOOKUP_SCAN>(acc, e, live, src, hot_lds);
    }
    if (live) store_ext(partial + t, acc);
    ZKP_WAVE_T1(4);
  }
}

struct msm_map {
  uint32_t N = 0, nc = 0;
  const uint32_t* order = nullptr;
};
__device__ __forceinline__ uint32_t msm_of_lane(const msm_map& m, uint32_t p) {
  if (!m.order) return p;
  const uint32_t q = p / m.N;
  return (p - q * m.N) * m.nc + m.order[q];
}

template <typename STATUS_T>
__global__ void __launch_bounds__(256, 2)
k_reduce_encode(uint32_t n_msm, const uint32_t* __restrict__ off, const uint32_t* __restrict__ pidx,
                uint32_t n_points, const dev_affine* __restrict__ pts, const dev_ext* __restrict__ partial,
                uint8_t* __restrict__ out, STATUS_T* __restrict__ status, const msm_map map) {
  const uint32_t lane = blockIdx.x * blockDim.x + threadIdx.x;
  if (lane >= n_msm) return;
  const uint32_t i = msm_of_lane(map, lane);
  const uint32_t b = off[i], e = off[i + 1];
  ge_p3 acc;
  ge_identity(acc);
  uint32_t bad = 0;
  if (b < e) load_ext(acc, partial + b);
#pragma unroll 1
  for (uint32_t t = b; t < e; ++t) {
    if (t != b) {
      ge_p3 q;
      load_ext(q, partial + t);
      ge_add_p3(acc, acc, q);
    }
    const uint32_t pi = pidx[t];
    bad |= pi < n_points ? (pts[pi].valid ^ 1u) : 1u;
  }
  uint32_t w[8];
  ristretto_encode(w, acc);
  if (bad) {
#pragma unroll
    for (int k = 0; k < 8; ++k) w[k] = 0;
  }
  store_vec<2>(out + 32 * (size_t)i, w);
  status[i] = (STATUS_T)bad;
}

__global__ void __launch_bounds__(256)
k_halve_scalars(uint32_t n, const uint8_t* __restrict__ in, uint8_t* __restrict__ out) {
  const uint32_t i = blockIdx.x * blockDim.x + threadIdx.x;
  if (i >= n) return;
  sc a, r;
  load_vec<2>(a.v, in + 32 * (size_t)i);
  sc_halve(r, a);
  store_vec<2>(out + 32 * (size_t)i, r.v);
}

constexpr int ENC_BLOCK = 256;
struct enc_tree { uint32_t node[2 * ENC_BLOCK][9]; };
__device__ __forceinline__ void tree_get(fe& r, const enc_tree& t, int n) {
#pragma unroll
  for (int i = 0; i < 9; ++i) r.v[i] = t.node[n][i];
  FE_TRACK(fe_set_ub_tight(r));
}
__device__ __forceinline__ void tree_put(enc_tree& t, int n, const fe& a) {
#pragma unroll
  for (int i = 0; i < 9; ++i) t.node[n][i] = a.v[i];
}
__device__ __forceinline__ void tree_up(enc_tree& t, int tid) {
  for (int w = ENC_BLOCK / 2; w >= 1; w >>= 1) {
    if (tid < w) {
      fe a, b, c;
      tree_get(a, t, 2 * (w + tid));
      tree_get(b, t, 2 * (w + tid) + 1);
      fe_mul(c, a, b);
      tree_put(t, w + tid, c);
    }
    __syncthreads();
  }
}
__device__ __forceinline__ void tree_down(enc_tree& t, int tid) {
  for (int w = 1; w <= ENC_BLOCK / 2; w <<= 1) {
    if (tid < w) {
      fe p, a, b, ia, ib;
      tree_get(p, t, w + tid);
      tree_get(a, t, 2 * (w + tid));
      tree_get(b, t, 2 * (w + tid) + 1);
      fe_mul(ia, p, b);
      fe_mul(ib, p, a);
      tree_put(t, 2 * (w + tid), ia);
      tree_put(t, 2 * (w + tid) + 1, ib);
    }
    __syncthreads();
  }
}

__device__ __forceinline__ uint32_t msm_sum(ge_p3& acc, uint32_t i, const uint32_t* __restrict__ off, const uint32_t* __restrict__ pidx,
                                            uint32_t n_points, const dev_affine* __restrict__ pts, const dev_ext* __restrict__ partial) {
  const uint32_t b = off[i], e = off[i + 1];
  ge_identity(acc);
  uint32_t bad = 0;
  if (b < e) load_ext(acc, partial + b);
#pragma unroll 1
  for (uint32_t t = b; t < e; ++t) {
    if (t != b) {
      ge_p3 q;
      load_ext(q, partial + t);
      ge_add_p3(acc, acc, q);
    }
    const uint32_t pi = pidx[t];
    bad |= pi < n_points ? (pts[pi].valid ^ 1u) : 1u;
  }
  return bad;
}

__device__ __forceinline__ void encode_invert_block(enc_tree& tree, int tid, uint32_t b, uint32_t n_blocks, const uint32_t* __restrict__ bprod,
                                                    uint32_t* __restrict__ binv) {
  fe x;
  fe_1(x);
  if (b < n_blocks) {
// ... 1037 lines not shown
#endif
void prof_begin(zkp_ctx* c) {
#ifdef ZKP_BUILD_TEST_HOOKS
  for (int64_t& v : c->sched) v = -1;
#endif
  c->n_ev = 0;
  if (c->profiling && !c->capturing) for (auto& s : c->kernel_names) s.clear();
  if (c->profiling && !c->capturing) { hipEventRecord(c->ev[0], c->stream); c->ev_kind[0] = -1; c->n_ev = 1; }
}
void prof_mark(zkp_ctx* c, int kind) {
  if (c->profiling && !c->capturing && !c->prof_suspended && c->n_ev < kMaxEvents) {
    hipEventRecord(c->ev[c->n_ev], c->stream);
    c->ev_kind[c->n_ev] = kind;
    c->n_ev++;
  }
}

inline dim3 grid1(size_t n, int block) { return dim3((unsigned)((n + block - 1) / block)); }
inline bool aligned16(const void* p) { return (reinterpret_cast<uintptr_t>(p) & 15) == 0; }

struct terms_cfg {
  int teeth = 4;
  uint32_t max_tables = 0xffffffffu, max_ladder = 0xffffffffu;
  bool throughput = false;
  uint32_t comb_min = 2;
  msm_map map;
  bool prehalved = false;
  stmt_job stmt;
  bool canonical = false;
  bool rider_tables = false;
};
inline bool stmt_classify_applies(const terms_cfg& k, uint32_t n_terms) {
  return k.stmt.on && n_terms >= 1024 && k.stmt.T <= STMT_MAX_TERMS && k.stmt.np <= STMT_MAX_POINTS && k.stmt.T && k.stmt.N;
}
inline terms_cfg terms_cfg_clamped(terms_cfg k, uint32_t n_points, uint32_t n_terms) {
  if (k.comb_min != 1) k.comb_min = 2;
  k.max_tables = std::min(k.max_tables, std::min(n_points, n_terms / k.comb_min));
  k.max_ladder = k.comb_min == 1 ? 0u : std::min(k.max_ladder, std::min(n_points, n_terms));
  if (k.teeth != 16) k.teeth = 4;
  return k;
}
constexpr uint64_t kThroughputEncodeMin = 2048;
inline int pick_teeth(uint64_t n_tab, uint64_t tab_terms) {
  if (!n_tab || tab_terms < 2 * n_tab) return 4;
  return n_tab * comb_entries(16) * sizeof(dev_ext) <= (64ull << 30) ? 16 : 4;
}

struct terms_layout { size_t pts, part, hot, cls, list, needs, slot_of, slot_pt, gstart, gfill, comb, ladder, half, states, xs, bprod, zflag, end; };
terms_layout terms_carve(size_t start, uint32_t n_points, uint32_t n_terms, uint32_t n_msm, const terms_cfg& k) {
  carve cv;
  cv.off = start;
  terms_layout o;
  const bool split = n_terms >= 1024;
  o.pts = cv.take((size_t)n_points * sizeof(dev_affine));
  o.part = cv.take((size_t)n_terms * sizeof(dev_ext));
  o.hot = cv.take((size_t)n_points * 4);
  o.cls = cv.take(512 * 4);
  o.needs = cv.take((size_t)n_points * 4);
  o.gfill = cv.take(split ? (size_t)n_points * 4 : 0);
  o.list = cv.take((size_t)n_terms * 4);
  o.slot_of = cv.take(split ? (size_t)n_points * 4 : 0);
  o.slot_pt = cv.take(split ? (size_t)k.max_tables * 4 : 0);
  o.gstart = cv.take(split ? (size_t)n_points * 4 : 0);
  o.comb = cv.take(split ? (size_t)k.max_tables * comb_entries(k.teeth) * sizeof(dev_ext) : 0);
  o.ladder = cv.take(split ? (((size_t)k.max_ladder + 63) / 64) * (k.stmt.pair ? 2 : 1) * LADDER_GROUP_UINT4 * sizeof(uint4) : 0);
  const uint32_t enc_blocks = (n_msm + ENC_BLOCK - 1) / ENC_BLOCK;
  o.half = cv.take(split ? (size_t)n_terms * 32 : 0);
  o.states = cv.take(split ? (size_t)n_msm * 54 * 4 : 0);
  o.xs = cv.take(split ? (size_t)n_msm * 9 * 4 : 0);
  o.bprod = cv.take(split ? (size_t)enc_blocks * 9 * 4 * 2 : 0);
  o.zflag = cv.take(split ? (size_t)n_msm : 0);
  o.end = cv.off;
  return o;
}
size_t terms_path_ws(uint32_t n_points, uint32_t n_terms, uint32_t n_msm, const terms_cfg& k = terms_cfg()) {
  return terms_carve(0, n_points, n_terms, n_msm, terms_cfg_clamped(k, n_points, n_terms)).end;
}

inline bool terms_batched_encode(const zkp_ctx* c, uint32_t n_terms, uint32_t n_msm, bool throughput) {
  return n_terms >= 1024 && (uint64_t)n_msm >= ((throughput && !c->batch_encode_user) ? kThroughputEncodeMin : c->batch_encode_min);
}

template <bool CT, int TEETH, int LOOKUP>
void launch_terms_split(zkp_ctx* c, dim3 grid, bool ladder, const uint8_t* d_scalars, const uint32_t* d_pidx, uint32_t n_points, const dev_ext* comb,
                        const uint32_t* slot_of, const uint32_t* class_start, const uint32_t* blk_start, const uint32_t* list,
                        const dev_affine* pts, dev_ext* ladder_rw, uint32_t max_ladder, dev_ext* part, uint32_t comb_split, const uint32_t* pair, uint32_t stmt_T,
                        uint32_t no_carry) {
  uint32_t stride = 0;
  const uint32_t lb = (max_ladder + 255) / 256;
  const bool interleave = ladder && lb && (c->ladder_interleave < 0 ? lb >= zkp_ctx::kInterleaveLadderBlocks : c->ladder_interleave != 0);
  if (ladder && lb) ZKP_SCHED(c, LADDER_INTERLEAVE, interleave);
  if (interleave) {
    stride = (grid.x / 2) / lb;
    if (stride % 2 == 0 && stride) --stride;
    if (stride < 2) stride = 0;
  }
  const bool split_kernel = CT && TEETH == 16 && LOOKUP == LOOKUP_XBAR && comb_split && !ladder;
  prof_note(c, ZKP_K_TERMS, std::string("k_terms_split<") + (CT ? "true" : "false") + ", " + std::to_string(TEETH) + ", " + (ladder ? "true" : "false") + ", " + std::to_string(LOOKUP) + ", " +
                            (split_kernel ? "true" : "false") + ">");
  if constexpr (CT && TEETH == 16 && LOOKUP == LOOKUP_XBAR) {
    if (comb_split && !ladder) {
      hipLaunchKernelGGL((k_terms_split<CT, TEETH, false, LOOKUP, true>), grid, dim3(256), 0, c->stream, d_scalars, d_pidx, n_points, comb, slot_of, class_start, blk_start, list,
                         c->hot_tables, pts, ladder_rw, max_ladder, part, stride, pair, stmt_T, no_carry);
      return;
    }
  }
  if (ladder)
    hipLaunchKernelGGL((k_terms_split<CT, TEETH, true, LOOKUP>), grid, dim3(256), 0, c->stream, d_scalars, d_pidx, n_points, comb, slot_of, class_start, blk_start, list,
                       c->hot_tables, pts, ladder_rw, max_ladder, part, stride, pair, stmt_T, no_carry);
  else
    hipLaunchKernelGGL((k_terms_split<CT, TEETH, false, LOOKUP>), grid, dim3(256), 0, c->stream, d_scalars, d_pidx, n_points, comb, slot_of, class_start, blk_start, list,
                       c->hot_tables, pts, ladder_rw, max_ladder, part, stride, pair, stmt_T, no_carry);
}

enum : int { PH_POINTS = 1, PH_SCALARS = 2, PH_ALL = 3 };
int msm_terms_path(zkp_ctx* c, uint32_t n_msm, const uint32_t* d_off, const uint8_t* d_scalars,
                   const uint32_t* d_pidx, const uint8_t* d_points, uint32_t n_points, uint32_t n_terms, int flags,
                   uint8_t* d_out, uint8_t* d_status8, uint32_t* d_status32, size_t ws_reserved, bool decode_all = false,
                   int phase = PH_ALL, const terms_cfg& cfg_in = terms_cfg()) {
  const terms_cfg k = terms_cfg_clamped(cfg_in, n_points, n_terms);
  const terms_layout o = terms_carve(ws_reserved, n_points, n_terms, n_msm, k);
  const bool batched_encode = terms_batched_encode(c, n_terms, n_msm, k.throughput);
  const uint32_t enc_blocks = (n_msm + ENC_BLOCK - 1) / ENC_BLOCK;
  if (o.end > c->ws_bytes) return fail(ZKP_ERR_ARG, "internal: workspace too small");
  const bool terms_split = n_terms >= 1024;
  const uint32_t enc_groups = (enc_blocks + ENC_BLOCK - 1) / ENC_BLOCK;
  if (phase & PH_SCALARS) {
    ZKP_SCHED(c, TERMS_SPLIT, terms_split);
    ZKP_SCHED(c, BATCH_ENCODE, batched_encode);
    if (batched_encode) ZKP_SCHED(c, ENC_GROUPS, enc_groups);
  }
  char* base = static_cast<char*>(c->ws);
  dev_affine* pts = reinterpret_cast<dev_affine*>(base + o.pts);
  dev_ext* part = reinterpret_cast<dev_ext*>(base + o.part);
  if (terms_split) {
    int32_t* hotmap = reinterpret_cast<int32_t*>(base + o.hot);
    uint32_t* cls = reinterpret_cast<uint32_t*>(base + o.cls);
    uint32_t* class_cnt = cls, *class_start = cls + 80, *cursor = cls + 160, *any_hot = cls + 240, *n_slots = cls + 241, *blk_start = cls + 256;
    uint32_t* list = reinterpret_cast<uint32_t*>(base + o.list);
    uint32_t* needs = reinterpret_cast<uint32_t*>(base + o.needs);
    uint32_t* slot_of = reinterpret_cast<uint32_t*>(base + o.slot_of);
    uint32_t* slot_pt = reinterpret_cast<uint32_t*>(base + o.slot_pt);
    dev_ext* comb = reinterpret_cast<dev_ext*>(base + o.comb);
    dev_ext* ladder = reinterpret_cast<dev_ext*>(base + o.ladder);
    const uint32_t comb_min = k.comb_min;
    const bool lat_split = c->comb_split < 0 ? (!k.throughput && flags == ZKP_CT && k.teeth == 16 && n_terms >= zkp_ctx::kSplitCombTerms && n_terms < zkp_ctx::kGroupedCombTerms) : c->comb_split != 0;
    const bool group_on = (HOT_LDS_ROWS && c->ct_lookup == LOOKUP_SCAN) ? false
                          : c->grouped_comb < 0 ? (n_terms >= (k.throughput ? zkp_ctx::kWideCallTerms : zkp_ctx::kGroupedCombTerms) || lat_split) : c->grouped_comb != 0;
    const bool comb_split = lat_split && flags == ZKP_CT && k.teeth == 16 && !(HOT_LDS_ROWS && c->ct_lookup != LOOKUP_XBAR);
    const uint32_t group_min = (flags == ZKP_CT && k.teeth == 16 && group_on && k.max_tables) ? GROUP_MIN_USES : 0xffffffffu;
    ZKP_SCHED(c, LAT_SPLIT, lat_split);
    ZKP_SCHED(c, GROUPED, group_on);
    ZKP_SCHED(c, COMB_MIN, comb_min);
    const bool pair_on = k.stmt.pair && flags == ZKP_VARTIME && stmt_classify_applies(k, n_terms);
    if (k.stmt.pair && !pair_on) return fail(ZKP_ERR_ARG, "paired terms outside the statement classifier");
    if (pair_on && !decode_all) return fail(ZKP_ERR_ARG, "paired terms need decode_all");
    const bool rider_ok = pair_on && k.teeth == 16 && k.rider_tables;
    if (pair_on) ZKP_SCHED(c, RIDERS, rider_ok);
    uint32_t* gstart = reinterpret_cast<uint32_t*>(base + o.gstart);
    uint32_t* gfill = reinterpret_cast<uint32_t*>(base + o.gfill);
    if ((phase & PH_POINTS) && stmt_classify_applies(k, n_terms)) {
      const size_t lanes = std::max<size_t>(std::max<size_t>(n_terms, n_points), (size_t)k.stmt.N * k.stmt.nc + 1);
      hipLaunchKernelGGL(k_stmt_classify, grid1(lanes, 256), dim3(256), 0, c->stream, k.stmt, d_points, c->hot_nreg, c->hot_reg_words, c->hot_reg_slot, comb_min, group_min,
                         k.max_tables, needs, class_start, blk_start, n_slots, slot_of, slot_pt, list, rider_ok ? 1u : 0u);
      prof_mark(c, ZKP_K_SORT);
      hipLaunchKernelGGL(k_decode_affine, grid1(n_points, 256), dim3(256), 0, c->stream, n_points, d_points, pts, decode_all ? (const uint32_t*)nullptr : needs);
      prof_mark(c, ZKP_K_DECODE);
    } else if (phase & PH_POINTS) {
    HIP_TRY(hipMemsetAsync(cls, 0, o.list - o.cls, c->stream));
    if (c->hot_nreg)
      hipLaunchKernelGGL(k_hot_match, grid1(n_points, 256), dim3(256), 0, c->stream, n_points, d_points, c->hot_nreg, c->hot_reg_words, c->hot_reg_slot, hotmap, any_hot);
    else
      HIP_TRY(hipMemsetAsync(hotmap, 0xff, (size_t)n_points * 4, c->stream));
    hipLaunchKernelGGL(k_use_count, grid1(n_terms, 256), dim3(256), 0, c->stream, n_terms, d_pidx, n_points, hotmap, needs);
    hipLaunchKernelGGL(k_class_count, grid1(n_terms, 256), dim3(256), 0, c->stream, n_terms, d_pidx, n_points, hotmap, needs, comb_min, group_min, class_cnt);
    prof_mark(c, ZKP_K_SORT);
    hipLaunchKernelGGL(k_decode_affine, grid1(n_points, 256), dim3(256), 0, c->stream, n_points, d_points, pts, decode_all ? (const uint32_t*)nullptr : needs);
    prof_mark(c, ZKP_K_DECODE);
    hipLaunchKernelGGL(k_class_scan, dim3(1), dim3(64), 0, c->stream, class_cnt, class_start, cursor, blk_start);
    if (k.max_tables)
      hipLaunchKernelGGL(k_comb_slots, grid1(n_points, 256), dim3(256), 0, c->stream, n_points, needs, comb_min, group_min, k.max_tables, n_slots, slot_of, slot_pt, gstart, pts);
    hipLaunchKernelGGL(k_class_scatter, grid1(n_terms, 256), dim3(256), 0, c->stream, n_terms, d_pidx, n_points, hotmap, needs, comb_min, group_min, class_start, gstart, gfill,
                       cursor, list);
    prof_mark(c, ZKP_K_SORT);
    }
    if ((phase & PH_POINTS) && k.max_tables) {
      if (c->tables_lane < 0 ? k.throughput : c->tables_lane != 0) {
        if (k.teeth == 16 && c->pending_tr.active) {
          const auto& t = c->pending_tr;
          const uint32_t tr_blocks = (t.N + TR_BLOCK / 2 - 1) / (TR_BLOCK / 2);
          if (t.steps) {
            const uint32_t rows = t.sd.n_img * 3u + ((t.sd.n_chk || (t.sd.tail >> 31)) ? 1u : 0u);
            if (rows) hipLaunchKernelGGL(k_transcript_assemble, dim3((t.N + TA_BLOCK - 1) / TA_BLOCK, rows), dim3(TA_BLOCK), 0, c->stream, t.sd, t.N, t.bufs, t.img, t.failed);
            hipLaunchKernelGGL(k_tables_chain_pc<16>, dim3((tr_blocks + 1) / 2 + (k.max_tables + 63) / 64), dim3(2 * TR_BLOCK), 0, c->stream, tr_blocks, t.sd,
                               reinterpret_cast<const uint32_t*>(t.img), t.N, t.bufs, t.ts, t.saved, n_slots, k.max_tables, slot_pt, pts, comb);
          } else
            hipLaunchKernelGGL(k_tables_transcript_pc<16>, dim3((tr_blocks + 1) / 2 + (k.max_tables + 63) / 64), dim3(2 * TR_BLOCK), 0, c->stream, tr_blocks, t.ops, t.n_ops,
                               t.tables, t.N, t.bufs, t.ts, t.saved, t.failed, t.tail, n_slots, k.max_tables, slot_pt, pts, comb);
          c->pending_tr.active = false;
          prof_note(c, ZKP_K_TABLES, t.steps ? "zkp::k_tables_chain_pc<16>" : "zkp::k_tables_transcript_pc<16>");
        } else if (k.teeth == 16) hipLaunchKernelGGL(k_comb_tables_lane<16>, grid1(k.max_tables, 256), dim3(256), 0, c->stream, n_slots, k.max_tables, slot_pt, pts, comb);
        else hipLaunchKernelGGL(k_comb_tables_lane<4>, grid1(k.max_tables, 256), dim3(256), 0, c->stream, n_slots, k.max_tables, slot_pt, pts, comb);
      } else {
        if (k.teeth == 16) hipLaunchKernelGGL(k_comb_tables<16>, grid1((size_t)k.max_tables * 4, 256), dim3(256), 0, c->stream, n_slots, k.max_tables, slot_pt, pts, comb);
        else hipLaunchKernelGGL(k_comb_tables<4>, grid1((size_t)k.max_tables * 4, 256), dim3(256), 0, c->stream, n_slots, k.max_tables, slot_pt, pts, comb);
      }
    }
    if ((phase & PH_POINTS) && k.max_tables && rider_ok)
      hipLaunchKernelGGL(k_rider_tables, grid1(k.max_tables, 256), dim3(256), 0, c->stream, n_slots, k.max_tables, slot_pt, pts, comb);
    if ((phase & PH_POINTS) && k.max_tables && c->kernel_names[ZKP_K_TABLES].find("k_tables_transcript") == std::string::npos && c->kernel_names[ZKP_K_TABLES].find("k_tables_chain") == std::string::npos)
      prof_note(c, ZKP_K_TABLES, std::string((c->tables_lane < 0 ? k.throughput : c->tables_lane != 0) ? "zkp::k_comb_tables_lane<" : "zkp::k_comb_tables<") + (k.teeth == 16 ? "16>" : "4>"));
    if (phase & PH_POINTS) prof_mark(c, ZKP_K_TABLES);
    const dim3 grid((unsigned)((n_terms + XBAR_BLOCK_TERMS - 1) / XBAR_BLOCK_TERMS + 4 + HOT_SLOTS + (comb_split ? 3 * ((n_terms + 255) / 256) + 1 : 0)));
    if (batched_encode) {
      uint8_t* d_half = reinterpret_cast<uint8_t*>(base + o.half);
      if (!k.prehalved) {
        if (phase & PH_SCALARS) hipLaunchKernelGGL(k_halve_scalars, grid1(n_terms, 256), dim3(256), 0, c->stream, n_terms, d_scalars, d_half);
        d_scalars = d_half;
      }
    }
    if (phase & PH_SCALARS) {
      const uint32_t no_carry = (k.canonical && flags == ZKP_CT) ? 1u : 0u;
      ZKP_SCHED(c, NO_CARRY, no_carry);
      const int lookup = (!HOT_LDS_ROWS || c->ct_lookup == LOOKUP_XBAR) ? LOOKUP_XBAR : (flags == ZKP_CT ? c->ct_lookup : LOOKUP_LDS);
      ZKP_SCHED(c, SIGN_FOLD, (no_carry && lookup == LOOKUP_XBAR) ? 1 : 0);
#define ZKP_LAUNCH_TERMS(CT_, TEETH_, LK_) launch_terms_split<CT_, TEETH_, LK_>(c, grid, k.max_ladder != 0, d_scalars, d_pidx, n_points, comb, slot_of, class_start, blk_start, list, pts, ladder, k.max_ladder, part, comb_split ? 1u : 0u, pair_on ? k.stmt.pair : (const uint32_t*)nullptr, k.stmt.T, no_carry)
      if (lookup == LOOKUP_XBAR) {
        if (flags == ZKP_CT) { if (k.teeth == 16) ZKP_LAUNCH_TERMS(true, 16, LOOKUP_XBAR); else ZKP_LAUNCH_TERMS(true, 4, LOOKUP_XBAR); }
        else { if (k.teeth == 16) ZKP_LAUNCH_TERMS(false, 16, LOOKUP_XBAR); else ZKP_LAUNCH_TERMS(false, 4, LOOKUP_XBAR); }
      }
#if ZKP_HOT_W <= 6
      else if (lookup == LOOKUP_SCAN) {
        if (k.teeth == 16) ZKP_LAUNCH_TERMS(true, 16, LOOKUP_SCAN); else ZKP_LAUNCH_TERMS(true, 4, LOOKUP_SCAN);
      } else {
        if (flags == ZKP_CT) { if (k.teeth == 16) ZKP_LAUNCH_TERMS(true, 16, LOOKUP_LDS); else ZKP_LAUNCH_TERMS(true, 4, LOOKUP_LDS); }
        else { if (k.teeth == 16) ZKP_LAUNCH_TERMS(false, 16, LOOKUP_LDS); else ZKP_LAUNCH_TERMS(false, 4, LOOKUP_LDS); }
      }
#endif
#undef ZKP_LAUNCH_TERMS
    }
  } else {
    if (n_points && (phase & PH_POINTS)) hipLaunchKernelGGL(k_decode_affine, grid1(n_points, 256), dim3(256), 0, c->stream, n_points, d_points, pts, (const uint32_t*)nullptr);
    prof_mark(c, ZKP_K_DECODE);
    if (n_terms && (phase & PH_SCALARS)) hipLaunchKernelGGL(k_terms_r4, grid1(n_terms, 256), dim3(256), 0, c->stream, n_terms, d_scalars, d_pidx, n_points, pts, part);
  }
  if (!(phase & PH_SCALARS)) { HIP_TRY(hipGetLastError()); return ZKP_OK; }
  prof_mark(c, ZKP_K_TERMS);
  if (n_msm && batched_encode) {
    uint32_t* states = reinterpret_cast<uint32_t*>(base + o.states);
    uint32_t* xs = reinterpret_cast<uint32_t*>(base + o.xs);
    uint32_t* bprod = reinterpret_cast<uint32_t*>(base + o.bprod);
    uint32_t* binv = bprod + (size_t)enc_blocks * 9;
    uint8_t* zflag = reinterpret_cast<uint8_t*>(base + o.zflag);
    if (d_status8)
      hipLaunchKernelGGL(k_encode_prepare<uint8_t>, dim3(enc_blocks), dim3(ENC_BLOCK), 0, c->stream, n_msm, d_off, d_pidx, n_points, pts, part, states, xs, bprod, zflag, d_status8, k.map);
    else
      hipLaunchKernelGGL(k_encode_prepare<uint32_t>, dim3(enc_blocks), dim3(ENC_BLOCK), 0, c->stream, n_msm, d_off, d_pidx, n_points, pts, part, states, xs, bprod, zflag, d_status32, k.map);
    hipLaunchKernelGGL(k_encode_invert, dim3(enc_groups), dim3(ENC_BLOCK), 0, c->stream, enc_blocks, bprod, binv);
    hipLaunchKernelGGL(k_encode_finish, dim3(enc_blocks), dim3(ENC_BLOCK), 0, c->stream, n_msm, d_off, d_pidx, n_points, pts, part, states, xs, binv, zflag,
                       (const uint8_t*)d_status8, (const uint32_t*)d_status32, d_out, k.map);
  } else if (n_msm) {
    if (d_status8)
      hipLaunchKernelGGL(k_reduce_encode<uint8_t>, grid1(n_msm, 256), dim3(256), 0, c->stream, n_msm, d_off, d_pidx, n_points, pts, part, d_out, d_status8, k.map);
    else
      hipLaunchKernelGGL(k_reduce_encode<uint32_t>, grid1(n_msm, 256), dim3(256), 0, c->stream, n_msm, d_off, d_pidx, n_points, pts, part, d_out, d_status32, k.map);
  }
  prof_mark(c, ZKP_K_REDUCE);
  HIP_TRY(hipGetLastError());
  return ZKP_OK;
}

inline uint32_t pip_part_len(uint64_t n) { return n < (1u << 18) ? 16u : (n < (1u << 21) ? 32u : 64u); }
template <int C>
size_t pip_vmax(uint64_t n) { return (size_t)(n / pip_part_len(n)) + pip_cfg<C>::B1 + 1; }

template <int C>
uint32_t pip_tiles(uint64_t n) { return (uint32_t)((n + sort_cfg<C>::TILE - 1) / sort_cfg<C>::TILE); }

template <int C>
size_t pip_ws(uint64_t n, uint32_t K = 1) {
  using cfg = pip_cfg<C>;
  const size_t WK = (size_t)cfg::W1 * K;
  carve cv;
  cv.take((size_t)K * n * sizeof(dev_niels));
  cv.take(WK * n * 4);
  cv.take(WK * n * 4);
  cv.take(WK * cfg::B1 * 4 * 3);
  cv.take(WK * (cfg::B1 + 1) * 4);
  cv.take(WK * pip_tiles<C>(n) * cfg::B1 * 4);
  cv.take(WK * pip_vmax<C>(n) * sizeof(dev_ext));
  cv.take(WK * pip_vmax<C>(n) * 4);
  cv.take((size_t)K * 4 + 256);
  cv.take(WK * cfg::B1 * sizeof(dev_ext));
  cv.take(WK * (cfg::B + 8) * sizeof(dev_ext) * 2);
  return cv.off;
}

template <int C>
int pip_run(zkp_ctx* c, uint32_t n, const uint8_t* d_scalars, const uint8_t* d_points, uint8_t* d_out,
            uint32_t* d_status, size_t ws_reserved, uint32_t* shared_flags, const pip_seg seg = pip_seg(), int phases = 3) {
  using cfg = pip_cfg<C>;
  const uint32_t K = seg.K;
  const size_t WK = (size_t)cfg::W1 * K;
  if (WK > 65535) return fail(ZKP_ERR_ARG, "too many batches in one call");
  carve cv;
  cv.off = ws_reserved;
  char* base = static_cast<char*>(c->ws);
  dev_niels* niels = reinterpret_cast<dev_niels*>(base + cv.take((size_t)K * n * sizeof(dev_niels)));
  uint32_t* digits = reinterpret_cast<uint32_t*>(base + cv.take(WK * n * 4));
  uint32_t* sorted = reinterpret_cast<uint32_t*>(base + cv.take(WK * n * 4));
  const size_t nb = WK * cfg::B1;
  if (nb * 4 > 0xffffffffull) return fail(ZKP_ERR_ARG, "too many batches in one call");
  uint32_t* hist = reinterpret_cast<uint32_t*>(base + cv.take(nb * 4 * 3));
  uint32_t* start = hist + nb;
  uint32_t* cursor = start + nb;
  uint32_t* vstart = reinterpret_cast<uint32_t*>(base + cv.take(WK * (cfg::B1 + 1) * 4));
  const uint32_t tiles = pip_tiles<C>(n);
  uint32_t* tilehist = reinterpret_cast<uint32_t*>(base + cv.take(WK * tiles * cfg::B1 * 4));
  const uint32_t L = pip_part_len(n);
  const size_t vmax = pip_vmax<C>(n);
  ZKP_SCHED(c, PIP_C, C);
  ZKP_SCHED(c, PIP_PART, L);
  dev_ext* parts = reinterpret_cast<dev_ext*>(base + cv.take(WK * vmax * sizeof(dev_ext)));
  uint32_t* vmap = reinterpret_cast<uint32_t*>(base + cv.take(WK * vmax * 4));
  uint32_t* invalid = reinterpret_cast<uint32_t*>(base + cv.take((size_t)K * 4 + 256));
  if (shared_flags) invalid = shared_flags;
  dev_ext* buckets = reinterpret_cast<dev_ext*>(base + cv.take(nb * sizeof(dev_ext)));
  const size_t lvl_cap = WK * (cfg::B + 8);
  dev_ext* lvlA = reinterpret_cast<dev_ext*>(base + cv.take(lvl_cap * sizeof(dev_ext) * 2));
  dev_ext* lvlR = lvlA + lvl_cap;
  if (cv.off > c->ws_bytes) return fail(ZKP_ERR_ARG, "internal: workspace too small");

  if (phases == 1) {
    if (!shared_flags) return fail(ZKP_ERR_ARG, "internal: split prepare without the caller's flag words");
    hipLaunchKernelGGL((k_pip_prepare<C, 1>), dim3((n + 255) / 256, K), dim3(256), 0, c->stream, n, seg, d_scalars, d_points, niels, digits, invalid);
    HIP_TRY(hipGetLastError());
    return ZKP_OK;
  }
  if (!shared_flags) HIP_TRY(hipMemsetAsync(invalid, 0, (size_t)K * 4, c->stream));
  prof_note(c, ZKP_K_DECODE, "k_pip_prepare<" + std::to_string(C) + ">");
  if (phases == 2) hipLaunchKernelGGL((k_pip_prepare<C, 2>), dim3((n + 255) / 256, K), dim3(256), 0, c->stream, n, seg, d_scalars, d_points, niels, digits, invalid);
  else hipLaunchKernelGGL((k_pip_prepare<C, 3>), dim3((n + 255) / 256, K), dim3(256), 0, c->stream, n, seg, d_scalars, d_points, niels, digits, invalid);
  prof_mark(c, ZKP_K_DECODE);
  hipLaunchKernelGGL(k_pip_tile_hist<C>, dim3(tiles, (unsigned)WK), dim3(sort_cfg<C>::THREADS), 0, c->stream, n, digits, tilehist);
  hipLaunchKernelGGL(k_pip_tile_total, grid1(nb, 256), dim3(256), 0, c->stream, cfg::B1, tiles, (uint32_t)nb, tilehist, hist);
  hipLaunchKernelGGL(k_pip_scan, dim3((unsigned)WK), dim3(256), 0, c->stream, cfg::B1, L, hist, start, cursor, vstart);
  hipLaunchKernelGGL(k_pip_tile_base, grid1(nb, 256), dim3(256), 0, c->stream, cfg::B1, tiles, (uint32_t)nb, start, tilehist);
  hipLaunchKernelGGL(k_pip_tile_scatter<C>, dim3(tiles, (unsigned)WK), dim3(sort_cfg<C>::THREADS), 0, c->stream, n, digits, tilehist, sorted);
  prof_mark(c, ZKP_K_SORT);
  hipLaunchKernelGGL(k_pip_vmap, grid1(nb, 256), dim3(256), 0, c->stream, cfg::B1, (uint32_t)nb, (uint32_t)vmax, vstart, vmap);
  hipLaunchKernelGGL(k_pip_bucket_part, dim3((unsigned)((vmax + 255) / 256), (unsigned)WK), dim3(256), 0, c->stream, n, (uint32_t)cfg::W1, cfg::B1, L, (uint32_t)vmax,
                     start, hist, vstart, vmap, sorted, niels, parts);
  constexpr size_t MERGE_LANE_MIN_BUCKETS = (size_t)1 << 19;
#ifdef ZKP_BUILD_TEST_HOOKS
  const bool lane_merge = c->debug_pip_merge ? c->debug_pip_merge == 2 : nb >= MERGE_LANE_MIN_BUCKETS;
#else
  const bool lane_merge = nb >= MERGE_LANE_MIN_BUCKETS;
#endif
  ZKP_SCHED(c, PIP_MERGE, lane_merge ? 1 : 0);
  ZKP_SCHED(c, PIP_BUCKETS, nb);
  if (lane_merge) hipLaunchKernelGGL(k_pip_bucket_merge<true>, grid1(nb, 256), dim3(256), 0, c->stream, cfg::B1, (uint32_t)nb, (uint32_t)vmax, vstart, parts, buckets);
  else hipLaunchKernelGGL(k_pip_bucket_merge<false>, grid1(nb * 4, 256), dim3(256), 0, c->stream, cfg::B1, (uint32_t)nb, (uint32_t)vmax, vstart, parts, buckets);
  prof_mark(c, ZKP_K_BUCKET);
  const dev_ext* Ain = nullptr;
  const dev_ext* Rin = buckets;
  uint32_t in_stride = cfg::B1, n_in = cfg::B;
  size_t lvl_off = 0;
  int level = 0;
  int shift = 0;
  static_assert(cfg::W1 <= 64, "k_pip_combine runs the last tree level with one quad per window in one 256-lane block");
  while (n_in > 1) {
    int lg = 0;
    while ((1u << lg) < n_in) ++lg;
    const int mbits = (level == 0 && lg % 3) ? lg % 3 : 3;
    const uint32_t m = 1u << mbits, n_out = n_in >> mbits;
// ... 1076 lines not shown
```

Baseline: 4.504 million.

## Fold scalar sign into comb recoding to drop carry entry and final tooth doublings

```diff
diff --git a/zkp_amd/csrc/comb_tables.h b/zkp_amd/csrc/comb_tables.h
--- a/zkp_amd/csrc/comb_tables.h
+++ b/zkp_amd/csrc/comb_tables.h
@@ -58,7 +58,7 @@
 template <int TEETH>
 __global__ void __launch_bounds__(256, 2)
 k_comb_tables(const uint32_t* __restrict__ n_slots, uint32_t max_tables, const uint32_t* __restrict__ slot_pt,
-              const dev_affine* __restrict__ pts, dev_ext* __restrict__ comb) {
+              const dev_affine* __restrict__ pts, dev_ext* __restrict__ comb, uint32_t no_carry) {
   using cfg = comb_cfg<TEETH>;
   const uint32_t gt = blockIdx.x * blockDim.x + threadIdx.x;
   const uint32_t slot = gt >> 2;
@@ -96,6 +96,7 @@
     q_to_cached(c, m, q); q_store_cached(tbl + 8 * j + 6, c, q);
     q_double(base, m4, q);
     q_to_cached(c, base, q); q_store_cached(tbl + 8 * j + 7, c, q);
+    if (no_carry && j == TEETH - 1) return;
 #pragma unroll 1
     for (int d = 0; d < cfg::BITS - 3; ++d) q_double(base, base, q);
   }
@@ -126,7 +127,7 @@
   }
   __builtin_amdgcn_wave_barrier();
 }
-template <int TEETH>
+template <int TEETH, bool NO_CARRY>
 __device__ __forceinline__ void comb_table_lane(uint32_t slot, const uint32_t* __restrict__ n_slots, uint32_t max_tables, const uint32_t* __restrict__ slot_pt,
                                                 const dev_affine* __restrict__ pts, dev_ext* __restrict__ comb) {
   using cfg = comb_cfg<TEETH>;
@@ -156,6 +157,7 @@
     ge_to_cached(c, m); store_comb_entry(tbl + 8 * j + 6, c);
     ge_double<true>(base, m4);
     ge_to_cached(c, base); store_comb_entry(tbl + 8 * j + 7, c);
+    if (NO_CARRY && j == TEETH - 1) return;
 #pragma unroll 1
     for (int d = 0; d < cfg::BITS - 4; ++d) ge_double<false>(base, base);
     ge_double<true>(base, base);
@@ -168,13 +170,19 @@
 __global__ void __launch_bounds__(256, 2)
 k_comb_tables_lane(const uint32_t* __restrict__ n_slots, uint32_t max_tables, const uint32_t* __restrict__ slot_pt,
                    const dev_affine* __restrict__ pts, dev_ext* __restrict__ comb) {
-  comb_table_lane<TEETH>(blockIdx.x * blockDim.x + threadIdx.x, n_slots, max_tables, slot_pt, pts, comb);
+  comb_table_lane<TEETH, false>(blockIdx.x * blockDim.x + threadIdx.x, n_slots, max_tables, slot_pt, pts, comb);
+}
+template <int TEETH>
+__global__ void __launch_bounds__(256, 2)
+k_comb_tables_lane_nc(const uint32_t* __restrict__ n_slots, uint32_t max_tables, const uint32_t* __restrict__ slot_pt,
+                      const dev_affine* __restrict__ pts, dev_ext* __restrict__ comb) {
+  comb_table_lane<TEETH, true>(blockIdx.x * blockDim.x + threadIdx.x, n_slots, max_tables, slot_pt, pts, comb);
 }
 
 
 template <int TEETH>
 __device__ __forceinline__ void comb_table_pc(uint32_t slot0, const uint32_t* __restrict__ n_slots, uint32_t max_tables, const uint32_t* __restrict__ slot_pt,
-                                              const dev_affine* __restrict__ pts, dev_ext* __restrict__ comb, uint32_t* hand) {
+                                              const dev_affine* __restrict__ pts, dev_ext* __restrict__ comb, uint32_t* hand, uint32_t no_carry) {
   using cfg = comb_cfg<TEETH>;
   const uint32_t wave = threadIdx.x >> 6, lane = threadIdx.x & 63u;
   const uint32_t ns = min(*n_slots, max_tables);
@@ -191,6 +199,7 @@
 #pragma unroll
       for (int i = 0; i < 9; ++i) { h[64 * i] = base.X.v[i]; h[64 * (9 + i)] = base.Y.v[i]; h[64 * (18 + i)] = base.Z.v[i]; h[64 * (27 + i)] = base.T.v[i]; }
       __syncthreads();
+      if (no_carry && j == TEETH - 1) return;
 #pragma unroll 1
       for (int d = 0; d < cfg::BITS - 1; ++d) ge_double<false>(base, base);
       ge_double<true>(base, base);
@@ -259,9 +268,12 @@
 __device__ __forceinline__ void term_comb(uint32_t t, const uint8_t* __restrict__ scalars, const dev_ext* __restrict__ tbl,
                                           dev_ext* __restrict__ partial, uint32_t* ecol, bool no_carry = false) {
   using cfg = comb_cfg<TEETH>;
-  uint32_t s[8], e[8], top;
+  static_assert(cfg::WINDOWS >= 2, "nibbles 62 and 63 are two windows of the last tooth");
+  const bool fold = CT && no_carry;
+  uint32_t s[8], e[8], top = 0, flip = 0;
   load_vec<2>(s, scalars + 32 * (size_t)t);
-  sc_add_pattern(e, top, s, 0x88888888u);
+  if (CT && fold) flip = sc_fold_recode16(e, s);
+  else sc_add_pattern(e, top, s, 0x88888888u);
 #pragma unroll
   for (int j = 0; j < 8; ++j) ecol[256 * j] = e[j];
   ge_p3 acc;
@@ -279,8 +291,9 @@
       for (int j = 0; j < TEETH; ++j) {
         const int nidx = j * cfg::WINDOWS + w;
         const uint32_t nib = (ecol[256 * (nidx >> 3)] >> (4 * (nidx & 7))) & 15u;
-        const uint32_t neg = (uint32_t)(nib < 8u);
-        const uint32_t mag = neg ? 8u - nib : nib - 8u;
+        const bool raw = fold && nidx == (int)SC_FOLD16_TOP_NIBBLE;
+        const uint32_t neg = raw ? 0u : (uint32_t)(nib < 8u);
+        const uint32_t mag = raw ? nib : (neg ? 8u - nib : nib - 8u);
         const dev_ext* row = tbl + 8 * j;
         ge_cached sel;
         ge_cached_identity(sel);
@@ -297,11 +310,13 @@
         const dev_ext* next = (j + 1 < TEETH) ? row + 8 : tbl;
         load_comb_entry(n0, next + 0);
         load_comb_entry(n1, next + 1);
+        if (fold && nidx == (int)SC_FOLD16_TOP_NIBBLE + 1) continue;
         ge_cached_cneg(sel, neg);
         if (w == cfg::WINDOWS - 1 && j == 0) ge_from_cached(acc, sel);
         else ge_add_cached(acc, acc, sel);
       }
     }
+    if (fold) ge_cneg(acc, flip);
   } else {
 #pragma unroll 1
     for (int w = cfg::WINDOWS - 1; w >= 0; --w) {
@@ -420,7 +435,7 @@
 
 __device__ __forceinline__ void comb_group_block(uint32_t i0, uint32_t n_g, const uint32_t* __restrict__ list_g, const uint8_t* __restrict__ scalars,
                                                  const uint32_t* __restrict__ pidx, const uint32_t* __restrict__ slot_of,
-                                                 const dev_ext* __restrict__ comb, dev_ext* __restrict__ partial, uint4* lds) {
+                                                 const dev_ext* __restrict__ comb, dev_ext* __restrict__ partial, uint4* lds, bool no_carry = false) {
   using cfg = comb_cfg<16>;
   constexpr uint32_t NONE = 0xffffffffu;
   const uint32_t tid = threadIdx.x, col = tid & 15u, k = tid >> 4;
@@ -515,9 +530,15 @@
   };
 #pragma unroll 1
   for (int pass = 0; pass < 2; ++pass) {
-    if (live && pass) { ge_double4(acc); ge_double4(lo); }
-    uint32_t alo = pass ? dlo[2] : dlo[3], ahi = pass ? dhi[2] : dhi[3];
-    uint32_t blo = pass ? dlo[0] : dlo[1], bhi = pass ? dhi[0] : dhi[1];
+    if (live && pass) {
+      ge_double4(acc);
+      ge_cached c;
+      ge_to_cached(c, lo);
+      ge_add_cached(acc, acc, c);
+      ge_double4(acc);
+    }
+    uint32_t alo = pass ? dlo[1] : dlo[3], ahi = pass ? dhi[1] : dhi[3];
+    uint32_t blo = pass ? dlo[0] : dlo[2], bhi = pass ? dhi[0] : dhi[2];
 #pragma unroll 1
     for (int j = 0; j < 16; ++j) {
       asm volatile("s_waitcnt vmcnt(0)\n\ts_barrier" ::: "memory");
@@ -535,26 +556,25 @@
       if (pass == 0 || j != 15) issue((uint32_t)((j + 1) & 15));
       if (live) {
         ge_cached_cneg(sel, neg);
-        if (first) ge_from_cached(lo, sel);
+        if (j == 0) ge_from_cached(lo, sel);
         else ge_add_cached(lo, lo, sel);
       }
     }
   }
   if (live) {
-    ge_double4(acc);
     ge_double4(acc);
     ge_cached c;
     ge_to_cached(c, lo);
     ge_add_cached(acc, acc, c);
   }
-  if (live) {
+  if (live && !no_carry) {
     ge_cached sel, c;
     ge_cached_identity(sel);
     load_comb_entry(c, comb + (size_t)slot * cfg::ENTRIES + 8 * 16);
     ge_cached_cmov(sel, c, top);
     ge_add_cached(acc, acc, sel);
-    store_ext(partial + t, acc);
-  }
+  }
+  if (live) store_ext(partial + t, acc);
 }
 
 constexpr uint32_t XBAR_RUNS = 8;
@@ -569,6 +589,7 @@
                                                 const uint32_t* __restrict__ pidx, const uint32_t* __restrict__ slot_of,
                                                 const dev_ext* __restrict__ comb, dev_ext* __restrict__ partial, uint4* lds, bool no_carry = false) {
   using cfg = comb_cfg<16>;
+  const bool fold = no_carry;
   constexpr uint32_t NONE = 0xffffffffu;
   const uint32_t tid = threadIdx.x, lane = tid & 63u;
   const uint32_t wave = (uint32_t)__builtin_amdgcn_readfirstlane((int)(tid >> 6));
@@ -611,13 +632,14 @@
       for (int q = 0; q < 9; ++q) __builtin_amdgcn_global_load_lds((gptr_t)(p + q), (lptr_t)(wlds + 64 * q), 16, 0, 0);
     }
   };
-  uint32_t dlo[cfg::WINDOWS], dhi[cfg::WINDOWS], top = 0;
+  uint32_t dlo[cfg::WINDOWS], dhi[cfg::WINDOWS], top = 0, flip = 0;
   {
     uint32_t sc[8], e[8];
 #pragma unroll
     for (int q = 0; q < 8; ++q) sc[q] = 0;
     if (live) load_vec<2>(sc, scalars + 32 * (size_t)t);
-    sc_add_pattern(e, top, sc, 0x88888888u);
+    if (fold) flip = sc_fold_recode16(e, sc);
+    else sc_add_pattern(e, top, sc, 0x88888888u);
 #pragma unroll
     for (int w = 0; w < cfg::WINDOWS; ++w) {
       uint32_t lo = 0, hi = 0;
@@ -634,12 +656,12 @@
   ge_identity(lo);
   issue(0);
   const uint32_t run8 = (run & (XBAR_RUNS - 1u)) * 8u;
-  auto pick = [&](uint32_t& c0, uint32_t& c1, ge_cached& sel, uint32_t& neg) {
+  auto pick = [&](uint32_t& c0, uint32_t& c1, ge_cached& sel, uint32_t& neg, bool raw) {
     const uint32_t nib = c0 & 15u;
     c0 = __builtin_amdgcn_alignbit(c1, c0, 4);
     c1 >>= 4;
-    neg = (uint32_t)(nib < 8u);
-    const uint32_t mag = neg ? 8u - nib : nib - 8u;
+    neg = raw ? 0u : (uint32_t)(nib < 8u);
+    const uint32_t mag = raw ? nib : (neg ? 8u - nib : nib - 8u);
     const uint32_t nz = (uint32_t)(mag != 0u);
     const int src = (int)((run8 + mag - nz) << 2);
     uint32_t wd[36];
@@ -657,34 +679,42 @@
   };
 #pragma unroll 1
   for (int pass = 0; pass < 2; ++pass) {
-    if (pass) { ge_double4(acc); ge_double4(lo); }
-    uint32_t alo = pass ? dlo[2] : dlo[3], ahi = pass ? dhi[2] : dhi[3];
-    uint32_t blo = pass ? dlo[0] : dlo[1], bhi = pass ? dhi[0] : dhi[1];
+    if (pass) {
+      ge_double4(acc);
+      ge_cached c;
+      ge_to_cached(c, lo);
+      ge_add_cached(acc, acc, c);
+      ge_double4(acc);
+    }
+    uint32_t alo = pass ? dlo[1] : dlo[3], ahi = pass ? dhi[1] : dhi[3];
+    uint32_t blo = pass ? dlo[0] : dlo[2], bhi = pass ? dhi[0] : dhi[2];
 #pragma unroll 1
     for (int j = 0; j < 16; ++j) {
       asm volatile("s_waitcnt vmcnt(0)" ::: "memory");
       ge_cached sel;
       uint32_t neg = 0;
-      const bool first = pass == 0 && j == 0;
-      pick(alo, ahi, sel, neg);
-      ge_cached_cneg(sel, neg);
-      if (first) ge_from_cached(acc, sel);
-      else ge_add_cached(acc, acc, sel);
-      pick(blo, bhi, sel, neg);
+      const bool top_tooth = fold && pass == 0 && j == 15;
+      if (!top_tooth) {
+        pick(alo, ahi, sel, neg, false);
+        ge_cached_cneg(sel, neg);
+        if (pass == 0 && j == 0) ge_from_cached(acc, sel);
+        else ge_add_cached(acc, acc, sel);
+      }
+      pick(blo, bhi, sel, neg, top_tooth);
       asm volatile("s_waitcnt lgkmcnt(0)" ::: "memory");
       if (pass == 0 || j != 15) issue((uint32_t)((j + 1) & 15));
       ge_cached_cneg(sel, neg);
-      if (first) ge_from_cached(lo, sel);
+      if (j == 0) ge_from_cached(lo, sel);
       else ge_add_cached(lo, lo, sel);
     }
   }
-  ge_double4(acc);
   ge_double4(acc);
   {
     ge_cached c;
     ge_to_cached(c, lo);
     ge_add_cached(acc, acc, c);
   }
+  if (fold) ge_cneg(acc, flip);
   if (live && !no_carry) {
     ge_cached sel, c;
     ge_cached_identity(sel);
@@ -732,9 +762,11 @@
 __device__ __forceinline__ void term_ladder16(uint32_t t, const uint8_t* __restrict__ scalars, const dev_affine* __restrict__ pt,
                                               uint4* __restrict__ tbl , dev_ext* __restrict__ partial, uint32_t* ecol,
                                               bool no_carry = false) {
-  uint32_t s[8], e[8], top;
+  const bool folded = CT && no_carry;
+  uint32_t s[8], e[8], top = 0, flip = 0;
   load_vec<2>(s, scalars + 32 * (size_t)t);
-  sc_add_pattern(e, top, s, 0x88888888u);
+  if (folded) flip = sc_fold_recode16(e, s);
+  else sc_add_pattern(e, top, s, 0x88888888u);
 #pragma unroll
   for (int j = 0; j < 8; ++j) ecol[256 * j] = e[j];
   ge_p3 acc;
@@ -766,11 +798,18 @@
       ge_from_cached(acc, sel);
     }
   }
+  if (folded) {
+    ge_cached sel;
+    ladder_select<CT>(sel, tbl, ecol[256 * 7] >> 24);
+    ge_from_cached(acc, sel);
+  }
 #pragma unroll 1
   for (int j = 7; j >= 0; --j) {
     uint32_t cur = ecol[256 * j];
-#pragma unroll 1
-    for (int k = 0; k < 8; ++k) {
+    int k = 0;
+    if (folded && j == 7) { cur <<= 8; k = 2; }
+#pragma unroll 1
+    for (; k < 8; ++k) {
       ge_double4(acc);
       const uint32_t nib = cur >> 28;
       cur <<= 4;
@@ -782,6 +821,7 @@
       ge_add_cached(acc, acc, sel);
     }
   }
+  if (folded) ge_cneg(acc, flip);
   store_ext(partial + t, acc);
 }
 
diff --git a/zkp_amd/csrc/fused_flows.h b/zkp_amd/csrc/fused_flows.h
--- a/zkp_amd/csrc/fused_flows.h
+++ b/zkp_amd/csrc/fused_flows.h
@@ -1011,6 +1011,7 @@
   if (o.end + terms_path_ws(n_points, N * T, N * nc, tk) > ws_bound)
     return fail(ZKP_ERR_ARG, "internal: prove_core's term path does not fit the workspace its caller sized");
   tk.throughput = throughput;
+  tk.canonical = true;
   if (pl.d_order) { tk.map.N = N; tk.map.nc = nc; tk.map.order = pl.d_order; }
   tk.stmt.toff = pl.d_tarr; tk.stmt.tpt = pl.d_tarr + nc + 1 + T; tk.stmt.N = N; tk.stmt.T = T; tk.stmt.nc = nc; tk.stmt.ns = pl.s.ns; tk.stmt.np = pl.s.np;
   tk.stmt.off = w.u32(o.off); tk.stmt.pidx = w.u32(o.pidx); tk.stmt.on = c->stmt_classify;
@@ -1042,7 +1043,6 @@
   prof_mark(c, ZKP_K_TRANSCRIPT);
 
   tk.prehalved = nc && terms_batched_encode(c, N * T, N * nc, tk.throughput);
-  tk.canonical = true;
   if (m && std::max(m, T) <= 256) {
     const uint32_t P = 256 / std::max(m, T);
     hipLaunchKernelGGL(k_blind_scalars, dim3((N + P - 1) / P), dim3(256), 0, c->stream, N, T, m, P, pl.d_tarr + nc + 1, w.u8(o.wide), w.u8(o.blind), w.u8(o.sc),
diff --git a/zkp_amd/csrc/sc25519.h b/zkp_amd/csrc/sc25519.h
--- a/zkp_amd/csrc/sc25519.h
+++ b/zkp_amd/csrc/sc25519.h
@@ -258,6 +258,22 @@
 #pragma unroll
   for (int i = 0; i < 8; ++i) s[i] = fold ? d[i] : s[i];
   return fold ? 1u : 0u;
+}
+
+constexpr uint32_t SC_FOLD16_TOP_NIBBLE = 62;
+ZKP_HD uint32_t sc_fold_recode16(uint32_t e[8], const uint32_t s[8]) {
+  uint32_t f[8];
+#pragma unroll
+  for (int i = 0; i < 8; ++i) f[i] = s[i];
+  const uint32_t flip = sc_fold_sign(f);
+  uint64_t c = 0;
+#pragma unroll
+  for (int i = 0; i < 8; ++i) {
+    c += (uint64_t)f[i] + (i < 7 ? 0x88888888u : 0x00888888u);
+    e[i] = (uint32_t)c;
+    c >>= 32;
+  }
+  return flip;
 }
 
 ZKP_HD void sc_halve(sc& r, const sc& a) {
diff --git a/zkp_amd/csrc/transcript_kernels.h b/zkp_amd/csrc/transcript_kernels.h
--- a/zkp_amd/csrc/transcript_kernels.h
+++ b/zkp_amd/csrc/transcript_kernels.h
@@ -296,7 +296,7 @@
 k_tables_transcript_pc(uint32_t tr_blocks, const tr_op* __restrict__ prog, uint32_t n_ops, const uint64_t* __restrict__ tables, uint32_t N, const tr_bufs bufs,
                        uint8_t* __restrict__ ts, uint32_t* __restrict__ saved, uint32_t* __restrict__ failed, uint32_t tail,
                        const uint32_t* __restrict__ n_slots, uint32_t max_tables, const uint32_t* __restrict__ slot_pt,
-                       const dev_affine* __restrict__ pts, dev_ext* __restrict__ comb) {
+                       const dev_affine* __restrict__ pts, dev_ext* __restrict__ comb, uint32_t no_carry) {
   __shared__ uint32_t S[2 * 36 * 64];
   static_assert(2 * 36 * 64 >= 2 * 25 * TR_BLOCK, "LDS of k_tables_transcript_pc");
   const uint32_t wave = threadIdx.x >> 6, trb = (tr_blocks + 1) / 2;
@@ -304,7 +304,7 @@
     const uint32_t bid = 2 * blockIdx.x + wave;
     if (bid < tr_blocks) transcript_pair_block(bid, S + wave * 25 * TR_BLOCK, prog, n_ops, tables, N, bufs, ts, saved, failed, tail);
   } else {
-    comb_table_pc<TEETH>((blockIdx.x - trb) * 64u, n_slots, max_tables, slot_pt, pts, comb, S);
+    comb_table_pc<TEETH>((blockIdx.x - trb) * 64u, n_slots, max_tables, slot_pt, pts, comb, S, no_carry);
   }
 }
 
@@ -312,14 +312,14 @@
 __global__ void __launch_bounds__(2 * TR_BLOCK, 2)
 k_tables_chain_pc(uint32_t tr_blocks, const tr_steps_dev p, const uint32_t* __restrict__ img32, uint32_t N, const tr_bufs bufs, uint8_t* __restrict__ ts,
                   uint32_t* __restrict__ saved, const uint32_t* __restrict__ n_slots, uint32_t max_tables, const uint32_t* __restrict__ slot_pt,
-                  const dev_affine* __restrict__ pts, dev_ext* __restrict__ comb) {
+                  const dev_affine* __restrict__ pts, dev_ext* __restrict__ comb, uint32_t no_carry) {
   __shared__ uint32_t S[2 * 36 * 64];
   const uint32_t wave = threadIdx.x >> 6, trb = (tr_blocks + 1) / 2;
   if (blockIdx.x < trb) {
     const uint32_t bid = 2 * blockIdx.x + wave;
     if (bid < tr_blocks) transcript_chain_block(bid, S + wave * 25 * TR_BLOCK, p, img32, N, bufs, ts, saved);
   } else {
-    comb_table_pc<TEETH>((blockIdx.x - trb) * 64u, n_slots, max_tables, slot_pt, pts, comb, S);
+    comb_table_pc<TEETH>((blockIdx.x - trb) * 64u, n_slots, max_tables, slot_pt, pts, comb, S, no_carry);
   }
 }
 
diff --git a/zkp_amd/csrc/zkp_kernels.hip b/zkp_amd/csrc/zkp_kernels.hip
--- a/zkp_amd/csrc/zkp_kernels.hip
+++ b/zkp_amd/csrc/zkp_kernels.hip
@@ -186,7 +186,7 @@
       if constexpr (LOOKUP == LOOKUP_XBAR)
         comb_group_xbar((vb - ladder_blocks - comb_blocks) * XBAR_BLOCK_TERMS, n_group, list + class_start[CLASS_GROUP], scalars, pidx, slot_of, comb, partial, hot_lds, no_carry != 0);
       else
-        comb_group_block((vb - ladder_blocks - comb_blocks) * 256u, n_group, list + class_start[CLASS_GROUP], scalars, pidx, slot_of, comb, partial, hot_lds);
+        comb_group_block((vb - ladder_blocks - comb_blocks) * 256u, n_group, list + class_start[CLASS_GROUP], scalars, pidx, slot_of, comb, partial, hot_lds, no_carry != 0);
     }
     ZKP_WAVE_T1(3);
   } else {
@@ -1530,6 +1530,7 @@
     ZKP_SCHED(c, LAT_SPLIT, lat_split);
     ZKP_SCHED(c, GROUPED, group_on);
     ZKP_SCHED(c, COMB_MIN, comb_min);
+    const uint32_t no_carry = (k.canonical && flags == ZKP_CT) ? 1u : 0u;
     const bool pair_on = k.stmt.pair && flags == ZKP_VARTIME && stmt_classify_applies(k, n_terms);
     if (k.stmt.pair && !pair_on) return fail(ZKP_ERR_ARG, "paired terms outside the statement classifier");
     if (pair_on && !decode_all) return fail(ZKP_ERR_ARG, "paired terms need decode_all");
@@ -1571,23 +1572,26 @@
             const uint32_t rows = t.sd.n_img * 3u + ((t.sd.n_chk || (t.sd.tail >> 31)) ? 1u : 0u);
             if (rows) hipLaunchKernelGGL(k_transcript_assemble, dim3((t.N + TA_BLOCK - 1) / TA_BLOCK, rows), dim3(TA_BLOCK), 0, c->stream, t.sd, t.N, t.bufs, t.img, t.failed);
             hipLaunchKernelGGL(k_tables_chain_pc<16>, dim3((tr_blocks + 1) / 2 + (k.max_tables + 63) / 64), dim3(2 * TR_BLOCK), 0, c->stream, tr_blocks, t.sd,
-                               reinterpret_cast<const uint32_t*>(t.img), t.N, t.bufs, t.ts, t.saved, n_slots, k.max_tables, slot_pt, pts, comb);
+                               reinterpret_cast<const uint32_t*>(t.img), t.N, t.bufs, t.ts, t.saved, n_slots, k.max_tables, slot_pt, pts, comb, no_carry);
           } else
             hipLaunchKernelGGL(k_tables_transcript_pc<16>, dim3((tr_blocks + 1) / 2 + (k.max_tables + 63) / 64), dim3(2 * TR_BLOCK), 0, c->stream, tr_blocks, t.ops, t.n_ops,
-                               t.tables, t.N, t.bufs, t.ts, t.saved, t.failed, t.tail, n_slots, k.max_tables, slot_pt, pts, comb);
+                               t.tables, t.N, t.bufs, t.ts, t.saved, t.failed, t.tail, n_slots, k.max_tables, slot_pt, pts, comb, no_carry);
           c->pending_tr.active = false;
           prof_note(c, ZKP_K_TABLES, t.steps ? "zkp::k_tables_chain_pc<16>" : "zkp::k_tables_transcript_pc<16>");
+        } else if (no_carry) {
+          if (k.teeth == 16) hipLaunchKernelGGL(k_comb_tables_lane_nc<16>, grid1(k.max_tables, 256), dim3(256), 0, c->stream, n_slots, k.max_tables, slot_pt, pts, comb);
+          else hipLaunchKernelGGL(k_comb_tables_lane_nc<4>, grid1(k.max_tables, 256), dim3(256), 0, c->stream, n_slots, k.max_tables, slot_pt, pts, comb);
         } else if (k.teeth == 16) hipLaunchKernelGGL(k_comb_tables_lane<16>, grid1(k.max_tables, 256), dim3(256), 0, c->stream, n_slots, k.max_tables, slot_pt, pts, comb);
         else hipLaunchKernelGGL(k_comb_tables_lane<4>, grid1(k.max_tables, 256), dim3(256), 0, c->stream, n_slots, k.max_tables, slot_pt, pts, comb);
       } else {
-        if (k.teeth == 16) hipLaunchKernelGGL(k_comb_tables<16>, grid1((size_t)k.max_tables * 4, 256), dim3(256), 0, c->stream, n_slots, k.max_tables, slot_pt, pts, comb);
-        else hipLaunchKernelGGL(k_comb_tables<4>, grid1((size_t)k.max_tables * 4, 256), dim3(256), 0, c->stream, n_slots, k.max_tables, slot_pt, pts, comb);
+        if (k.teeth == 16) hipLaunchKernelGGL(k_comb_tables<16>, grid1((size_t)k.max_tables * 4, 256), dim3(256), 0, c->stream, n_slots, k.max_tables, slot_pt, pts, comb, no_carry);
+        else hipLaunchKernelGGL(k_comb_tables<4>, grid1((size_t)k.max_tables * 4, 256), dim3(256), 0, c->stream, n_slots, k.max_tables, slot_pt, pts, comb, no_carry);
       }
     }
     if ((phase & PH_POINTS) && k.max_tables && rider_ok)
       hipLaunchKernelGGL(k_rider_tables, grid1(k.max_tables, 256), dim3(256), 0, c->stream, n_slots, k.max_tables, slot_pt, pts, comb);
     if ((phase & PH_POINTS) && k.max_tables && c->kernel_names[ZKP_K_TABLES].find("k_tables_transcript") == std::string::npos && c->kernel_names[ZKP_K_TABLES].find("k_tables_chain") == std::string::npos)
-      prof_note(c, ZKP_K_TABLES, std::string((c->tables_lane < 0 ? k.throughput : c->tables_lane != 0) ? "zkp::k_comb_tables_lane<" : "zkp::k_comb_tables<") + (k.teeth == 16 ? "16>" : "4>"));
+      prof_note(c, ZKP_K_TABLES, std::string((c->tables_lane < 0 ? k.throughput : c->tables_lane != 0) ? (no_carry ? "zkp::k_comb_tables_lane_nc<" : "zkp::k_comb_tables_lane<") : "zkp::k_comb_tables<") + (k.teeth == 16 ? "16>" : "4>"));
     if (phase & PH_POINTS) prof_mark(c, ZKP_K_TABLES);
     const dim3 grid((unsigned)((n_terms + XBAR_BLOCK_TERMS - 1) / XBAR_BLOCK_TERMS + 4 + HOT_SLOTS + (comb_split ? 3 * ((n_terms + 255) / 256) + 1 : 0)));
     if (batched_encode) {
@@ -1598,7 +1602,6 @@
       }
     }
     if (phase & PH_SCALARS) {
-      const uint32_t no_carry = (k.canonical && flags == ZKP_CT) ? 1u : 0u;
       ZKP_SCHED(c, NO_CARRY, no_carry);
       const int lookup = (!HOT_LDS_ROWS || c->ct_lookup == LOOKUP_XBAR) ? LOOKUP_XBAR : (flags == ZKP_CT ? c->ct_lookup : LOOKUP_LDS);
       ZKP_SCHED(c, SIGN_FOLD, (no_carry && lookup == LOOKUP_XBAR) ? 1 : 0);
```

Result: faster. 4.608 million, median of 6 (+2.3%).
